# vlongle/pixie

Measured on NVIDIA H100. Metric: unet_voxels_per_s, higher is better.
Workload: dtype fp16e5 (U-Net, fp32 accumulate) + f32 (MPM)

## Files before the change

### pixie_b200/csrc/capi.cu

```cuda
#include "../../include/pixie_b200.h"
#include "mpm.cuh"
#include "unet.cuh"
#include "unet_kernels.cuh"
#include "field_transfer.cuh"
#include "cluster.cuh"
#include "particle_fill.cuh"
#include "nearest.cuh"
#include "gs_render.cuh"
#include "gs_ply.cuh"
#include "gs_load.cuh"
#include "material_metrics.cuh"
#include "part_segmentation.cuh"
#include "workspace.cuh"

#include <algorithm>
#include <cstring>
#include <string>

namespace {
thread_local std::string g_err;
}

namespace pixie {
int fail(const std::string& message) { g_err = message; return 1; }
int fail(const std::string& what, cudaError_t e) {
    cudaGetLastError();
    return fail(what + ": " + cudaGetErrorString(e));
}
}

using pixie::fail;

namespace {
int check(const char* op, cudaError_t e) { return e == cudaSuccess ? 0 : fail(op, e); }
}

extern "C" {

const char* pixie_last_error(void) { return g_err.c_str(); }
int pixie_abi_version(void) { return 2; }

int pixie_device_ok(void) {
    int dev = 0;
    if (cudaGetDevice(&dev) != cudaSuccess) { cudaGetLastError(); return 0; }
    int major = 0;
    if (cudaDeviceGetAttribute(&major, cudaDevAttrComputeCapabilityMajor, dev) != cudaSuccess) { cudaGetLastError(); return 0; }
    return major == 9 ? 1 : 0;
}

static int require_device() {
    if (!pixie_device_ok()) return fail("pixie_b200 requires an sm_90 (H100) CUDA device; there is no CPU fallback");
    return 0;
}

int pixie_unet_create(const pixie_unet_config* cfg, pixie_unet_t* out) {
    if (!cfg || !out) return fail("null argument");
    if (require_device()) return 1;
    *out = pixie::unet_create(*cfg);
    return *out ? 0 : 1;
}
int pixie_unet_set_tensor(pixie_unet_t h, const char* name, const float* host_data, const int64_t* shape, int ndim) {
    if (!h || !name || !host_data) return fail("null argument");
    return pixie::unet_set_tensor(h, name, host_data, shape, ndim);
}
int pixie_unet_finalize(pixie_unet_t h) {
    if (!h) return fail("null handle");
    return pixie::unet_finalize(h);
}
int pixie_unet_forward(pixie_unet_t h, const void* feat, int batch, float* out, void* stream) {
    if (!h || !feat || !out) return fail("null argument");
    return pixie::unet_forward(h, feat, batch, out, (cudaStream_t)stream);
}
int pixie_unet_forward_ncdhw(pixie_unet_t h, const float* feat, int batch, float* out, void* stream) {
    if (!h || !feat || !out) return fail("null argument");
    return pixie::unet_forward_ncdhw(h, feat, batch, out, (cudaStream_t)stream);
}
int pixie_unet_forward_host(pixie_unet_t h, const void* feat, int batch, float* out, void* stream) {
    if (!h || !feat || !out) return fail("null argument");
    return pixie::unet_forward_host(h, feat, batch, out, (cudaStream_t)stream);
}
int pixie_unet_profile(pixie_unet_t h, const void* feat, int batch, float* out, void* stream, float* ms, int* kinds, double* flops, int cap) {
    if (!h || !feat || !out || !ms || !kinds || !flops) { fail("null argument"); return -1; }
    return pixie::unet_profile(h, feat, batch, out, (cudaStream_t)stream, ms, kinds, flops, cap);
}
int pixie_field_extract(const float* pred, int n_classes, const float* mask, int D, const double ranges[6], const double bmin[3], const double bmax[3],
                        float* pos, float* density, float* E, float* nu, int* material, float* conf, int* count_host, void* stream) {
    if (!pred || !mask || !ranges || !bmin || !bmax || !pos || !density || !E || !nu || !material || !conf || !count_host) return fail("null argument");
    if (D < 2 || D > 1290 || n_classes < 1)
        return fail("field_extract: need 2 <= D <= 1290 (D^3 voxels are indexed in int32) and at least one class channel");
    if (require_device()) return 1;
    return check("field_extract", pixie::field_extract(pred, n_classes, mask, D, ranges, bmin, bmax, pos, density, E, nu, material, conf,
                                                       count_host, (cudaStream_t)stream));
}
int pixie_knn_assign(const float* query, int nq, const float* pos, const float* density, const float* E, const float* nu, const int* material,
                     const int* part, const float* conf, int m, int k, double threshold, int weighted, const float defaults[4], int def_material,
                     int def_part, float* o_density, float* o_E, float* o_nu, int* o_material, int* o_part, float* o_conf, int* n_too_far_host,
                     void* stream) {
    if (!query || !pos || !density || !E || !nu || !material || !part || !conf || !defaults || !o_density || !o_E || !o_nu || !o_material ||
        !o_part || !o_conf || !n_too_far_host) return fail("null argument");
    if (k < 1 || k > 16) return fail("knn_assign: k must be in [1, 16]");
    if (m < 1) return fail("knn_assign: empty material point cloud");
    if (k > m) return fail("knn_assign: k exceeds the number of material points");
    if (require_device()) return 1;
    return check("knn_assign", pixie::knn_assign(query, nq, pos, density, E, nu, material, part, conf, m, k, threshold, weighted, defaults,
                                                 def_material, def_part, o_density, o_E, o_nu, o_material, o_part, o_conf, n_too_far_host,
                                                 (cudaStream_t)stream));
}
int pixie_dbscan(const float* pos, int n, const int* ids, int select_id, double eps, int min_samples, int* index, int* labels,
                 int* n_selected_host, int* n_clusters_host, void* stream) {
    if (!n_selected_host || !n_clusters_host || (n > 0 && (!pos || !index || !labels))) return fail("null argument");
    if (n < 0) return fail("dbscan: negative point count");
    if (!(eps > 0.0) || min_samples < 1) return fail("dbscan: need eps > 0 and min_samples >= 1");
    if (require_device()) return 1;
    return check("dbscan", pixie::dbscan(pos, n, ids, select_id, eps, min_samples, index, labels, n_selected_host, n_clusters_host,
                                         (cudaStream_t)stream));
}
int pixie_cluster_stats(const float* pos, const int* index, const int* labels, int n_selected, int n_clusters, int* sizes,
                        float* bbox_min, float* bbox_max, void* stream) {
    if (n_selected < 0 || n_clusters < 0) return fail("cluster_stats: negative count");
    if ((n_selected > 0 && (!pos || !index || !labels)) || (n_clusters > 0 && (!sizes || !bbox_min || !bbox_max))) return fail("null argument");
    if (require_device()) return 1;
    return check("cluster_stats", pixie::cluster_stats(pos, index, labels, n_selected, n_clusters, sizes, bbox_min, bbox_max, (cudaStream_t)stream));
}
int pixie_particle_volume(const float* pos, int n, int grid_n, float grid_dx, float* vol, void* stream) {
    if (n < 0) return fail("particle_volume: negative point count");
    if (n > 0 && (!pos || !vol)) return fail("null argument");
    if (grid_n < 1 || !(grid_dx > 0.f)) return fail("particle_volume: bad grid");
    if (require_device()) return 1;
    return check("particle_volume", pixie::particle_volume(pos, n, grid_n, grid_dx, vol, (cudaStream_t)stream));
}
int pixie_frame_transform(const float* pos, const float* cov, int n, float z_shift, float scale, const float mean[3], const float* rotations,
                          int n_rot, float* pos_out, float* cov_out, void* stream) {
    if (n < 0) return fail("frame_transform: negative point count");
    if (!mean || (n > 0 && (!pos || !pos_out || (cov && !cov_out))) || (n_rot > 0 && !rotations)) return fail("null argument");
    if (n_rot < 0 || n_rot > 8) return fail("frame_transform: at most 8 rotations");
    if (require_device()) return 1;
    return check("frame_transform", pixie::frame_transform(pos, cov, n, z_shift, scale, mean, rotations, n_rot, pos_out, cov_out, (cudaStream_t)stream));
}
int pixie_gaussian_ply_records(const float* pos, const float* cov, const float* shs, int K, const float* opacity, int n, float* records,
                               void* stream) {
    if (n < 0) return fail("gaussian_ply_records: negative point count");
    if (K != 1 && K != 4 && K != 9 && K != 16) return fail("gaussian_ply_records: K must be 1, 4, 9 or 16 SH coefficients");
    if (n > 0 && (!pos || !cov || !shs || !opacity || !records)) return fail("null argument");
    if (require_device()) return 1;
    return check("gaussian_ply_records", pixie::gaussian_ply_records(pos, cov, shs, K, opacity, n, records, (cudaStream_t)stream));
}
int pixie_gaussian_checkpoint_decode(const void* table, long long n, int row_bytes, const int* cols, int K, int has_threshold, float threshold,
                                     float* pos, float* shs, float* opacity, float* cov, long long* m_host, void* stream) {
    if (!cols || !m_host || (n > 0 && (!table || !pos || !shs || !opacity || !cov))) return fail("null argument");
    if (n < 0) return fail("gaussian_checkpoint_decode: negative row count");
    if (K != 1 && K != 4 && K != 9 && K != 16) return fail("gaussian_checkpoint_decode: K must be 1, 4, 9 or 16 SH coefficients");
    if (row_bytes < 4 || row_bytes % 4 != 0 || row_bytes / 4 > pixie::kGsLoadMaxRowWords)
        return fail("gaussian_checkpoint_decode: the row stride must be a multiple of 4 bytes, at most " +
                       std::to_string(4 * pixie::kGsLoadMaxRowWords));
    const int row_words = row_bytes / 4, n_cols = 11 + 3 * K;
    pixie::GsColumns c{};
    int* dst[59];
    int k = 0;
    for (int i = 0; i < 3; ++i) dst[k++] = &c.xyz[i];
    for (int i = 0; i < 3; ++i) dst[k++] = &c.dc[i];
    for (int i = 0; i < 3 * (K - 1); ++i) dst[k++] = &c.rest[i];
    dst[k++] = &c.opacity;
    for (int i = 0; i < 3; ++i) dst[k++] = &c.scale[i];
    for (int i = 0; i < 4; ++i) dst[k++] = &c.rot[i];
    for (int i = 0; i < n_cols; ++i) {
        if (cols[i] < 0 || cols[i] % 4 != 0 || cols[i] / 4 >= row_words)
            return fail("gaussian_checkpoint_decode: column " + std::to_string(i) + " is not a 4-byte aligned offset inside the row");
        *dst[i] = cols[i] / 4;
    }
    if (require_device()) return 1;
    return check("gaussian_checkpoint_decode", pixie::gaussian_checkpoint_decode(table, n, row_words, c, K, has_threshold, threshold, pos, shs, opacity,
                                                                                 cov, m_host, (cudaStream_t)stream));
}
int pixie_material_metrics(const float* mat, int c_mat, const float* mask, const float* seg, int n_classes, const float* cont, int n,
                           int64_t voxels, const double* ranges, int background_id, float* gt, long long* counts, double* sums, void* stream) {
    if (!ranges || (n > 0 && (!mat || !seg || !cont || !gt || !counts || !sums))) return fail("null argument");
    if (n < 0 || voxels < 1) return fail("material_metrics: need n >= 0 samples of at least one voxel");
    if (c_mat < 4) return fail("material_metrics: the material grid needs at least 4 channels (density, E, nu, ..., material id)");
    if (n_classes < 1) return fail("material_metrics: need at least one class");
    pixie::MaterialNorm nm;
    for (int c = 0; c < 3; ++c) {
        const double lo = ranges[2 * c], hi = ranges[2 * c + 1];
        nm.lo[c] = (float)lo;
        nm.hi[c] = (float)hi;
        nm.span[c] = (float)(hi - lo);
    }
    if (require_device()) return 1;
    return check("material_metrics", pixie::material_metrics(mat, c_mat, mask, seg, n_classes, cont, n, voxels, nm, background_id, gt, counts, sums,
                                                             (cudaStream_t)stream));
}
static bool fill_grid_ok(int grid_n) { return grid_n >= 1 && grid_n <= 1290; }
int pixie_fill_density(const float* pos, const float* opacity, const float* cov, int n, int grid_n, float grid_dx, int* count, float* density,
                       void* stream) {
    if (!count || !density || (n > 0 && (!pos || !opacity || !cov))) return fail("null argument");
    if (n < 0 || !fill_grid_ok(grid_n) || !(grid_dx > 0.f)) return fail("fill_density: need n >= 0, 1 <= grid_n <= 1290 and grid_dx > 0");
    if (require_device()) return 1;
    return check("fill_density", pixie::fill_density(pos, opacity, cov, n, grid_n, grid_dx, count, density, (cudaStream_t)stream));
}
int pixie_fill_grids(int* count, const float* density, int grid_n, float grid_dx, const float origin[3], float density_thres, float search_thres,
                     int max_particles_per_cell, int exclude_dir, int ray_cast_dir, unsigned long long seed, float* out, int max_samples,
                     int* n_dense_host, int* n_total_host, void* stream) {
    if (!count || !density || !origin || !n_dense_host || !n_total_host || (max_samples > 0 && !out)) return fail("null argument");
    if (!fill_grid_ok(grid_n) || !(grid_dx > 0.f)) return fail("fill_grids: need 1 <= grid_n <= 1290 and grid_dx > 0");
    if (max_particles_per_cell < 1 || (long long)grid_n * grid_n * grid_n * max_particles_per_cell > 2147483647LL)
        return fail("fill_grids: need 1 <= max_particles_per_cell and grid_n^3 * max_particles_per_cell < 2^31");
    if (exclude_dir < 0 || exclude_dir > 5 || ray_cast_dir < 0 || ray_cast_dir > 5) return fail("fill_grids: directions must be in 0..5");
    if (max_samples < 0) return fail("fill_grids: negative max_samples");
    if (require_device()) return 1;
    if (check("fill_grids", pixie::fill_grids(count, density, grid_n, grid_dx, origin, density_thres, search_thres, max_particles_per_cell,
                                              exclude_dir, ray_cast_dir, seed, out, max_samples, n_dense_host, n_total_host, (cudaStream_t)stream)))
        return 1;
    if (*n_total_host > max_samples)
        return fail("fill_grids: filling adds " + std::to_string(*n_total_host) + " particles (" + std::to_string(*n_dense_host) +
                       " in dense cells) but max_samples is " + std::to_string(max_samples));
    return 0;
}
int pixie_nearest_gaussian(const float* pos, int n, const float* query, int m, int* index, void* stream) {
    if (n < 0 || m < 0) return fail("nearest_gaussian: negative count");
    if ((n > 0 && m > 0 && !pos) || (m > 0 && (!query || !index))) return fail("null argument");
    if (require_device()) return 1;
    return check("nearest_gaussian", pixie::nearest_gaussian(pos, n, query, m, index, (cudaStream_t)stream));
}
int pixie_nearest_vertex(const double* vert, int n, const float* query, int m, int* index, void* stream) {
    if (n < 0 || m < 0) return fail("nearest_vertex: negative count");
    if ((n > 0 && m > 0 && !vert) || (m > 0 && (!query || !index))) return fail("null argument");
    if (require_device()) return 1;
    return check("nearest_vertex", pixie::nearest_vertex(vert, n, query, m, index, (cudaStream_t)stream));
}
int pixie_knn_label_vote(const float* pos, int n, const int64_t* labels, int k, int64_t* out, void* stream) {
    if (n < 0) return fail("knn_label_vote: negative count");
    if (n > 0 && (k < 1 || k > n)) return fail("knn_label_vote: k must be in [1, n]");
    if (n > 0 && (!pos || !labels || !out)) return fail("null argument");
    if (require_device()) return 1;
    return check("knn_label_vote", pixie::knn_label_vote(pos, n, (const long long*)labels, k, (long long*)out, (cudaStream_t)stream));
}
int pixie_part_similarity(const void* feat, const uint8_t* mask, int64_t n_voxels, int C, int n_occupied, const float* query, int P,
                          float inv_temperature, float* sims, int64_t* labels, float* scores, float* probs, void* stream) {
    if (n_voxels < 0 || n_occupied < 0) return fail("part_similarity: negative count");
    if (n_voxels > INT32_MAX) return fail("part_similarity: more than 2^31 - 1 voxels");
    if (C < 1) return fail("part_similarity: C must be >= 1");
    if (P < 1 || P > pixie::kMaxParts) return fail("part_similarity: P must be in [1, " + std::to_string(pixie::kMaxParts) + "]");
    if (n_occupied > n_voxels) return fail("part_similarity: more occupied voxels than voxels");
    if (n_occupied > 0 && (!feat || !query || !sims || !labels || !scores)) return fail("null argument");
    if (require_device()) return 1;
    return check("part_similarity", pixie::part_similarity((const __half*)feat, mask, n_voxels, C, n_occupied, query, P, inv_temperature,
                                                           sims, labels, scores, probs, (cudaStream_t)stream));
}
int pixie_gs_renderer_create(pixie_gs_renderer_t* out) {
    if (!out) return fail("null argument");
    if (require_device()) return 1;
    *out = pixie::gs_renderer_create();
    return *out ? 0 : 1;
}
int pixie_gs_render(pixie_gs_renderer_t h, const float* means, const float* cov, const float* opacity, const float* shs, int sh_coeffs,
                    int sh_degree, const float* colors, int n, const float view[16], const float proj[16], const float campos[3],
                    float tan_fovx, float tan_fovy, int width, int height, const float bg[3], float* image, int* radii, int* n_rendered,
                    float* phase_ms, void* stream) {
    if (!h) return fail("null handle");
    if (!view || !proj || !campos || !bg || !image || (n > 0 && (!means || !cov || !opacity || !radii || (!shs && !colors))))
        return fail("null argument");
    if (n < 0) return fail("gs_render: negative Gaussian count");
    if (width < 1 || height < 1 || (long long)width * height > 2147483647LL) return fail("gs_render: bad image size");
    if (!(tan_fovx > 0.f) || !(tan_fovy > 0.f)) return fail("gs_render: tan(fov) must be positive");
    if (shs && (sh_degree < 0 || sh_degree > 3 || (sh_degree + 1) * (sh_degree + 1) > sh_coeffs))
        return fail("gs_render: need 0 <= sh_degree <= 3 and (sh_degree + 1)^2 <= sh_coeffs");
    pixie::GsRenderArgs a{};
    a.means = means; a.cov = cov; a.opacity = opacity; a.shs = shs; a.colors = shs ? nullptr : colors;
    a.n = n; a.sh_coeffs = sh_coeffs; a.sh_degree = sh_degree;
    std::memcpy(a.view, view, sizeof(a.view));
    std::memcpy(a.proj, proj, sizeof(a.proj));
    std::memcpy(a.campos, campos, sizeof(a.campos));
    std::memcpy(a.bg, bg, sizeof(a.bg));
    a.tan_fovx = tan_fovx; a.tan_fovy = tan_fovy; a.width = width; a.height = height; a.image = image; a.radii = radii;
    return pixie::gs_render(h, a, n_rendered, phase_ms, (cudaStream_t)stream);
}
void pixie_gs_renderer_destroy(pixie_gs_renderer_t h) { pixie::gs_renderer_destroy(h); }
int pixie_pack_predictions(const float* seg_logits_dev, const float* cont_dev, float* out_dev, int batch, int64_t voxels, int n_classes, void* stream) {
    if (!seg_logits_dev || !cont_dev || !out_dev) return fail("null argument");
    if (require_device()) return 1;
    return check("pack_predictions",
                 (cudaError_t)pixie::launch_pack_predictions(seg_logits_dev, cont_dev, out_dev, batch, voxels, n_classes, (cudaStream_t)stream));
}
int pixie_unet_launch_count(pixie_unet_t h) { return h ? pixie::unet_launch_count(h) : 0; }
double pixie_unet_flops(pixie_unet_t h) { return h ? pixie::unet_flops(h) : 0.0; }
int pixie_unet_check(pixie_unet_t h) {
    if (!h) return fail("null handle");
    return pixie::unet_check(h);
}
int64_t pixie_unet_debug_fetch(pixie_unet_t h, const char* name, float* host_out, int64_t capacity) {
    if (!h || !name) { fail("null argument"); return -1; }
    return pixie::unet_debug_fetch(h, name, host_out, capacity);
}
int64_t pixie_unet_debug_names(pixie_unet_t h, char* buf, int64_t capacity) {
    if (!h || (!buf && capacity > 0)) { fail("null argument"); return -1; }
    const std::string s = pixie::unet_debug_names(h);
    if (capacity > 0) {
        const size_t n = std::min(s.size(), (size_t)capacity - 1);
        memcpy(buf, s.data(), n);
        buf[n] = '\0';
    }
    return (int64_t)s.size();
}
void pixie_unet_destroy(pixie_unet_t h) { pixie::unet_destroy(h); }

int pixie_mpm_create(int n_particles, int n_grid, float grid_lim, pixie_mpm_t* out) {
    if (!out) return fail("null argument");
    if (require_device()) return 1;
    *out = pixie::mpm_create(n_particles, n_grid, grid_lim);
    return *out ? 0 : 1;
}
int pixie_mpm_bind(pixie_mpm_t h, int field, void* dev_ptr) { return h ? pixie::mpm_bind(h, field, dev_ptr) : fail("null handle"); }
int pixie_mpm_set_params(pixie_mpm_t h, const pixie_mpm_params* p) { return !p ? fail("null params") : h ? pixie::mpm_set_params(h, *p) : fail("null handle"); }
int pixie_mpm_add_bc(pixie_mpm_t h, const pixie_mpm_bc* bc) { return !bc ? fail("null bc") : h ? pixie::mpm_add_bc(h, *bc) : fail("null handle"); }
int pixie_mpm_clear_bcs(pixie_mpm_t h) { return h ? pixie::mpm_clear_bcs(h) : fail("null handle"); }
int pixie_mpm_set_time(pixie_mpm_t h, double t) { return h ? pixie::mpm_set_time(h, t) : fail("null handle"); }
int pixie_mpm_get_time(pixie_mpm_t h, double* t) { return h ? pixie::mpm_get_time(h, t) : fail("null handle"); }
int pixie_mpm_step(pixie_mpm_t h, int n, double dt, void* stream) { return h ? pixie::mpm_step(h, n, dt, (cudaStream_t)stream) : fail("null handle"); }
int pixie_mpm_compute_mu_lam(pixie_mpm_t h, void* s) { return h ? pixie::mpm_compute_mu_lam(h, (cudaStream_t)s) : fail("null handle"); }
int pixie_mpm_compute_bulk(pixie_mpm_t h, void* s) { return h ? pixie::mpm_compute_bulk(h, (cudaStream_t)s) : fail("null handle"); }
int pixie_mpm_compute_mass(pixie_mpm_t h, void* s) { return h ? pixie::mpm_compute_mass(h, (cudaStream_t)s) : fail("null handle"); }
int pixie_mpm_compute_cov_from_F(pixie_mpm_t h, void* s) { return h ? pixie::mpm_compute_cov_from_F(h, (cudaStream_t)s) : fail("null handle"); }
int pixie_mpm_compute_R_from_F(pixie_mpm_t h, void* s) { return h ? pixie::mpm_compute_R_from_F(h, (cudaStream_t)s) : fail("null handle"); }
int pixie_mpm_apply_additional_params(pixie_mpm_t h, const float* boxes, int n_boxes, void* s) {
    return h ? pixie::mpm_apply_additional_params(h, boxes, n_boxes, (cudaStream_t)s) : fail("null handle");
}
int pixie_mpm_select_box(pixie_mpm_t h, const float point[3], const float size[3], int* mask, void* s) {
    return h ? pixie::mpm_select_box(h, point, size, mask, (cudaStream_t)s) : fail("null handle");
}
int pixie_mpm_select_cylinder(pixie_mpm_t h, const float point[3], const float normal[3], float hh, float radius, int* mask, void* s) {
    return h ? pixie::mpm_select_cylinder(h, point, normal, hh, radius, mask, (cudaStream_t)s) : fail("null handle");
}
int pixie_mpm_sync(pixie_mpm_t h, void* s) { return h ? pixie::mpm_sync(h, (cudaStream_t)s) : fail("null handle"); }
int pixie_mpm_set_active_count(pixie_mpm_t h, int n_active) { return h ? pixie::mpm_set_active_count(h, n_active) : fail("null handle"); }
int pixie_mpm_grid_ptrs(pixie_mpm_t h, float** mv4, float** v4) { return h ? pixie::mpm_grid_ptrs(h, mv4, v4) : fail("null handle"); }
int pixie_mpm_exchange_buffer(pixie_mpm_t h, void** base, size_t* bytes) { return h ? pixie::mpm_exchange_buffer(h, base, bytes) : fail("null handle"); }
int pixie_mpm_slab_attach(pixie_mpm_t h, int x0, int x1, int slack, const void* left, const void* right) {
    return h ? pixie::mpm_slab_attach(h, x0, x1, slack, left, right) : fail("null handle");
}
int pixie_mpm_slab_phase(pixie_mpm_t h, int phase, double dt, void* s) { return h ? pixie::mpm_slab_phase(h, phase, dt, (cudaStream_t)s) : fail("null handle"); }
int pixie_mpm_slab_error(pixie_mpm_t h, int* flag) { return h ? pixie::mpm_slab_error(h, flag) : fail("null handle"); }
int pixie_mpm_slab_excursion(pixie_mpm_t h, int* d_out, void* s) { return h ? pixie::mpm_slab_excursion(h, d_out, (cudaStream_t)s) : fail("null handle"); }
int pixie_ipc_export(const void* dev_ptr, unsigned char handle[64]) {
    static_assert(sizeof(cudaIpcMemHandle_t) == 64, "cudaIpcMemHandle_t size");
    cudaIpcMemHandle_t hd;
    if (check("cudaIpcGetMemHandle", cudaIpcGetMemHandle(&hd, const_cast<void*>(dev_ptr)))) return 1;
    memcpy(handle, &hd, 64);
    return 0;
}
int pixie_ipc_open(const unsigned char handle[64], void** dev_ptr) {
    cudaIpcMemHandle_t hd;
    memcpy(&hd, handle, 64);
    return check("cudaIpcOpenMemHandle", cudaIpcOpenMemHandle(dev_ptr, hd, cudaIpcMemLazyEnablePeerAccess));
}
int pixie_ipc_close(void* dev_ptr) { return check("cudaIpcCloseMemHandle", cudaIpcCloseMemHandle(dev_ptr)); }
long long pixie_mpm_launch_count(pixie_mpm_t h) { return h ? pixie::mpm_launch_count(h) : 0; }
void pixie_mpm_destroy(pixie_mpm_t h) { pixie::mpm_destroy(h); }

}
```

### pixie_b200/csrc/conv3d_igemm.cu

```cuda
#include "conv3d_igemm.cuh"
#include "ptx.cuh"

#include <algorithm>
#include <cmath>
#include <cstdio>
#include <cstring>

#include <cuda_fp8.h>

namespace pixie {

using namespace ptx;

namespace {

constexpr int kMaxWStages = 4;
constexpr int kMaxSStages = 8;
constexpr int kConsumerWarps = 8;
constexpr int kProducerWarp = 8;

struct SmemCtrl {
    uint64_t wfull[kMaxWStages];
    uint64_t wempty[kMaxWStages];
    uint64_t sfull[kMaxSStages];
    uint64_t sempty[kMaxSStages];
    int abort_flag;
};

constexpr int kCtlBarrierBytes = 512;
constexpr int kCmChunk = 16;
constexpr int kCmStageLd = 68;
constexpr int kCmStageFloats = kCmChunk * kCmStageLd;
constexpr int kStatsMaxC = 256;

struct TileCoord {
    int nb, d0, h0, w0, n0, ph_begin, ph_end, split, tde;
};

__device__ __forceinline__ TileCoord decode_tile(const ConvKernelParams& p, int wi) {
    TileCoord t;
    unsigned rest = (unsigned)wi;
    if (p.split_k == 1) {
        t.split = 0; t.ph_begin = 0; t.ph_end = p.n_phases;
    } else {
        const unsigned sk = (unsigned)p.split_k;
        t.split = (int)(rest % sk);
        rest /= sk;
        t.ph_begin = (int)(((unsigned)t.split * (unsigned)p.n_phases) / sk);
        t.ph_end = (int)((((unsigned)t.split + 1u) * (unsigned)p.n_phases) / sk);
    }
    const unsigned nt = rest % (unsigned)p.n_tiles;
    unsigned m = rest / (unsigned)p.n_tiles;
    const unsigned tw = m % (unsigned)p.tiles_w;
    m /= (unsigned)p.tiles_w;
    const unsigned th = m % (unsigned)p.tiles_h;
    m /= (unsigned)p.tiles_h;
    const unsigned td = m % (unsigned)p.tiles_d;
    t.nb = (int)(m / (unsigned)p.tiles_d);
    t.d0 = (int)td * p.TD;
    t.h0 = (int)th * p.TH;
    t.w0 = (int)tw * p.TW;
    t.n0 = (int)nt * p.block_n;
    t.tde = min(p.TD, p.D - t.d0);
    return t;
}

template <int N, bool F8>
__device__ __forceinline__ void mma_block(float* acc, uint32_t a, uint32_t b) {
    wgmma_fence();
#pragma unroll
    for (int k4 = 0; k4 < 4; ++k4) {
        const uint64_t da = make_sw128_desc(a + 32u * k4), db = make_sw128_desc(b + 32u * k4);
        if (F8) {
            if (N == 16) wgmma_e5m2_n16(acc, da, db);
            if (N == 32) wgmma_e5m2_n32(acc, da, db);
            if (N == 64) wgmma_e5m2_n64(acc, da, db);
            if (N == 128) wgmma_e5m2_n128(acc, da, db);
            if (N == 256) wgmma_e5m2_n256(acc, da, db);
        } else {
            if (N == 16) wgmma_f16_n16(acc, da, db);
            if (N == 32) wgmma_f16_n32(acc, da, db);
            if (N == 64) wgmma_f16_n64(acc, da, db);
            if (N == 128) wgmma_f16_n128(acc, da, db);
            if (N == 256) wgmma_f16_n256(acc, da, db);
        }
    }
    wgmma_commit();
}

__device__ __forceinline__ void wgmma_wait_n(int n) {
    switch (n) {
        case 0: wgmma_wait<0>(); break;
        case 1: wgmma_wait<1>(); break;
        case 2: wgmma_wait<2>(); break;
        case 3: wgmma_wait<3>(); break;
        case 4: wgmma_wait<4>(); break;
        case 5: wgmma_wait<5>(); break;
        case 6: wgmma_wait<6>(); break;
        case 7: wgmma_wait<7>(); break;
        case 8: wgmma_wait<8>(); break;
        case 9: wgmma_wait<9>(); break;
        default: wgmma_wait<0>(); break;
    }
}

struct RingPos {
    int stage = 0, parity = 0;
    __device__ __forceinline__ void advance(int n_stages) {
        if (++stage == n_stages) { stage = 0; parity ^= 1; }
    }
};

struct PendingStages {
    int s = -1, w = -1;
    __device__ __forceinline__ void release(SmemCtrl* ctl, int lane) {
        if (lane == 0) {
            if (s >= 0) mbar_arrive(&ctl->sempty[s]);
            if (w >= 0) mbar_arrive(&ctl->wempty[w]);
        }
        s = -1; w = -1;
    }
};

struct ConvStats {
    float* rows;
    int nb = -1;
    double tot_s = 0.0, tot_q = 0.0;

    __device__ __forceinline__ void flush(const ConvKernelParams& p, int lane) {
        if (p.stats_scalar) {
#pragma unroll
            for (int off = 16; off >= 1; off >>= 1) {
                tot_s += __shfl_xor_sync(0xffffffffu, tot_s, off);
                tot_q += __shfl_xor_sync(0xffffffffu, tot_q, off);
            }
            if (lane == 0) {
                atomicAdd(p.stats + (size_t)nb * p.Cout * 2, tot_s);
                atomicAdd(p.stats + (size_t)nb * p.Cout * 2 + 1, tot_q);
            }
            tot_s = 0.0; tot_q = 0.0;
            return;
        }
        asm volatile("bar.sync 1, 256;" ::: "memory");
        for (int ch = threadIdx.x; ch < p.Cout; ch += 256) {
            atomicAdd(p.stats + ((size_t)nb * p.Cout + ch) * 2, (double)rows[ch]);
            atomicAdd(p.stats + ((size_t)nb * p.Cout + ch) * 2 + 1, (double)rows[p.stats_ld + ch]);
            rows[ch] = 0.f;
            rows[p.stats_ld + ch] = 0.f;
        }
        asm volatile("bar.sync 1, 256;" ::: "memory");
    }
    __device__ __forceinline__ void enter(const ConvKernelParams& p, int item_nb, int lane) {
        if (nb != item_nb) {
            if (nb >= 0) flush(p, lane);
            nb = item_nb;
        }
    }
};

struct ConvSmem {
    uint8_t* w;
    uint8_t* s;
    SmemCtrl* ctl;
    float* stage;
    float* stats;
};

__device__ __forceinline__ ConvSmem conv_prologue(const ConvKernelParams& p, int stage_floats, int n_threads) {
    extern __shared__ __align__(1024) uint8_t smem_raw[];
    uint8_t* smem = reinterpret_cast<uint8_t*>(
        (reinterpret_cast<uintptr_t>(smem_raw) + 1023) & ~static_cast<uintptr_t>(1023));
    ConvSmem m;
    m.w = smem;
    m.s = smem + (size_t)p.w_stages * p.w_stage_bytes;
    m.ctl = reinterpret_cast<SmemCtrl*>(m.s + (size_t)p.s_stages * p.s_stage_bytes);
    m.stage = reinterpret_cast<float*>(reinterpret_cast<uint8_t*>(m.ctl) + kCtlBarrierBytes);
    m.stats = m.stage + stage_floats;
    const bool smem_misaligned = (p.smem_slack == 0) && (smem != smem_raw);

    if (threadIdx.x == 0) {
        for (int i = 0; i < kMaxWStages; ++i) { mbar_init(&m.ctl->wfull[i], 1); mbar_init(&m.ctl->wempty[i], kConsumerWarps); }
        for (int i = 0; i < kMaxSStages; ++i) { mbar_init(&m.ctl->sfull[i], 1); mbar_init(&m.ctl->sempty[i], kConsumerWarps); }
        m.ctl->abort_flag = smem_misaligned ? 1 : 0;
        fence_barrier_init();
    }
    if ((threadIdx.x >> 5) == kProducerWarp && (threadIdx.x & 31) == 0) {
        for (int i = 0; i < kConvMaxSrc; ++i) prefetch_tmap(&p.tmA[i]);
        prefetch_tmap(&p.tmB);
    }
    if (p.stats != nullptr && !p.stats_scalar)
        for (int i = threadIdx.x; i < 2 * p.stats_ld; i += n_threads) m.stats[i] = 0.f;
    __syncthreads();
    return m;
}

__device__ __forceinline__ void conv_report_abort(const ConvKernelParams& p, const SmemCtrl* ctl) {
    __syncthreads();
    if (threadIdx.x == 0 && ctl->abort_flag && p.err_flag) atomicExch(p.err_flag, 1 + (int)blockIdx.x);
}

template <int BN, int TD>
__device__ __forceinline__ int issue_slab(float (&acc)[TD][BN / 2], uint32_t a_addr, uint32_t w_addr, int pl, int d_min, int d_max,
                                          int n_kd, int n_kh, int TW, bool f8) {
    int groups = 0;
#pragma unroll
    for (int d = 0; d < TD; ++d) {
        if (d < d_min || d > d_max) continue;
        const int kd = pl - d;
        for (int kh = 0; kh < n_kh; ++kh) {
            const uint32_t a = a_addr + (uint32_t)(kh * TW * 128);
            const uint32_t b = w_addr + (uint32_t)(conv_wtile(0, n_kd, kh, kd) * BN * 128);
            if (f8) mma_block<BN, true>(acc[d], a, b);
            else mma_block<BN, false>(acc[d], a, b);
            ++groups;
        }
    }
    return groups;
}

constexpr int kWholePhase = 0;

template <int kUnitKd>
__device__ __forceinline__ void produce_tiles(const ConvKernelParams& p, SmemCtrl* ctl, uint8_t* w_smem, uint8_t* s_smem,
                                              volatile int* abort_flag, int total_items) {
    RingPos wring, sring;
    bool ok = true;
    for (int wi = blockIdx.x; wi < total_items && ok; wi += gridDim.x) {
        const TileCoord t = decode_tile(p, wi);
        for (int ph = t.ph_begin; ph < t.ph_end && ok; ++ph) {
            const ConvPhase P = p.phases[ph];
            const int n_kd = P.n_kd, n_kh = P.n_kh, nplanes = t.tde + n_kd - 1;
            const int unit_kd = kUnitKd ? kUnitKd : n_kd, n_units = kUnitKd ? n_kd / kUnitKd : 1;
            const uint32_t slab_bytes = (uint32_t)p.slab_rows[P.src] * 128u, unit_bytes = (uint32_t)(n_kh * unit_kd * p.block_n * 128);
            const CUtensorMap* tm = &p.tmA[P.src];
            const int cw = t.w0 * p.stride + P.dw, ch = t.h0 * p.stride + P.dh0, cd = t.d0 * p.stride + P.dd0;
#pragma unroll 1
            for (int pl = 0; pl < nplanes && ok; ++pl) {
                if (pl < n_units) {
                    ok = mbar_wait(&ctl->wempty[wring.stage], wring.parity ^ 1, abort_flag);
                    if (!ok) break;
                    if (elect_one()) {
                        mbar_expect_tx(&ctl->wfull[wring.stage], unit_bytes);
                        uint8_t* wdst = w_smem + (size_t)wring.stage * p.w_stage_bytes;
                        const int kd_lo = pl * unit_kd, kd_hi = kd_lo + unit_kd - 1;
#pragma unroll 1
                        for (int kh = 0; kh < n_kh; ++kh)
                            for (int kd = kd_hi; kd >= kd_lo; --kd)
                                tma_load_2d(wdst + (size_t)conv_wtile(0, unit_kd, kh, kd - kd_lo) * p.block_n * 128, &p.tmB,
                                            &ctl->wfull[wring.stage], conv_wtile(P.wtile_base, n_kd, kh, kd) * 64, t.n0);
                    }
                    wring.advance(p.w_stages);
                }
                ok = mbar_wait(&ctl->sempty[sring.stage], sring.parity ^ 1, abort_flag);
                if (!ok) break;
                if (elect_one()) {
                    mbar_expect_tx(&ctl->sfull[sring.stage], slab_bytes);
                    tma_load_5d(s_smem + (size_t)sring.stage * p.s_stage_bytes, tm, &ctl->sfull[sring.stage], (int)P.c0, cw, ch,
                                cd + pl * p.stride, t.nb);
                }
                sring.advance(p.s_stages);
            }
        }
    }
}

}

template <int BN, int TD>
__global__ void __launch_bounds__(kConvThreads, 1)
conv3d_igemm_kernel(const __grid_constant__ ConvKernelParams p) {
    const ConvSmem sm = conv_prologue(p, 0, kConvThreads);
    SmemCtrl* ctl = sm.ctl;
    volatile int* abort_flag = &ctl->abort_flag;
    const int warp = threadIdx.x >> 5;
    const int lane = threadIdx.x & 31;
    const int total_items = conv_work_items(p.NB, p.tiles_d, p.tiles_h, p.tiles_w, p.n_tiles, p.split_k);
    const bool do_stats = p.stats != nullptr;
    const bool scalar_stats = do_stats && p.stats_scalar;

    if (warp == kProducerWarp) {
        produce_tiles<kWholePhase>(p, ctl, sm.w, sm.s, abort_flag, total_items);
    } else {
        const int g = warp >> 2, wq = warp & 3;
        float acc[TD][BN / 2];
        RingPos wring, sring;
        const uint32_t w_base0 = smem_u32(sm.w), s_base0 = smem_u32(sm.s) + (uint32_t)(g * 64 * 128);
        bool ok = true;
        const long long DHW = (long long)p.D * p.H * p.W;
        ConvStats stats{sm.stats};
        int th2[2], tw2[2];
#pragma unroll
        for (int r2 = 0; r2 < 2; ++r2) {
            const int r = g * 64 + wq * 16 + (lane >> 2) + 8 * r2;
            th2[r2] = r / p.TW; tw2[r2] = r % p.TW;
        }
        const int cq = (lane & 3) * 2;

        for (int wi = blockIdx.x; wi < total_items && ok; wi += gridDim.x) {
            const TileCoord t = decode_tile(p, wi);
#pragma unroll
            for (int d = 0; d < TD; ++d)
#pragma unroll
                for (int j = 0; j < BN / 2; ++j) acc[d][j] = 0.f;
            PendingStages pend;
            int prev_f8 = -1;
            for (int ph = t.ph_begin; ph < t.ph_end && ok; ++ph) {
                const ConvPhase P = p.phases[ph];
                const int n_kd = P.n_kd, n_kh = P.n_kh;
                const bool f8 = P.f8 != 0;
                if (prev_f8 >= 0 && prev_f8 != (int)f8) wgmma_wait<0>();
                prev_f8 = (int)f8;
                ok = mbar_wait(&ctl->wfull[wring.stage], wring.parity, abort_flag);
                if (!ok) break;
                const uint32_t w_addr = w_base0 + (uint32_t)(wring.stage * p.w_stage_bytes);
                const int nplanes = t.tde + n_kd - 1;
                for (int pl = 0; pl < nplanes && ok; ++pl) {
                    ok = mbar_wait(&ctl->sfull[sring.stage], sring.parity, abort_flag);
                    if (!ok) break;
                    const int d_min = max(0, pl - (n_kd - 1)), d_max = min(t.tde - 1, pl);
                    const int groups = issue_slab<BN, TD>(acc, s_base0 + (uint32_t)(sring.stage * p.s_stage_bytes), w_addr, pl, d_min,
                                                          d_max, n_kd, n_kh, p.TW, f8);
                    wgmma_wait_n(groups);
                    pend.release(ctl, lane);
                    pend.s = sring.stage;
                    sring.advance(p.s_stages);
                }
                pend.w = wring.stage;
                wring.advance(p.w_stages);
                if (p.w_stages == 1) { wgmma_wait<0>(); pend.release(ctl, lane); }
            }
            wgmma_wait<0>();
            pend.release(ctl, lane);
#pragma unroll
            for (int d = 0; d < TD; ++d)
#pragma unroll
                for (int j = 0; j < BN / 2; ++j) fence_operand(acc[d][j]);
            if (!ok) break;

            if (do_stats) stats.enter(p, t.nb, lane);
            const bool first_split = (t.split == 0);
            const bool use_bias = first_split && p.bias != nullptr;
            const bool use_res = first_split && p.residual != nullptr;
#pragma unroll
            for (int d = 0; d < TD; ++d) {
                if (d >= t.tde) break;
#pragma unroll
                for (int r2 = 0; r2 < 2; ++r2) {
                    const int hh = t.h0 + th2[r2], ww = t.w0 + tw2[r2];
                    const bool row_ok = (hh < p.H) && (ww < p.W);
                    const long long vox = ((long long)(t.d0 + d) * p.H + hh) * p.W + ww;
#pragma unroll
                    for (int j8 = 0; j8 < BN / 8; ++j8) {
                        const int ch = t.n0 + j8 * 8 + cq;
                        float& a0 = acc[d][j8 * 4 + r2 * 2];
                        float& a1 = acc[d][j8 * 4 + r2 * 2 + 1];
                        const bool ok0 = row_ok && ch < p.Cout, ok1 = row_ok && ch + 1 < p.Cout;
                        float v0 = a0, v1 = a1;
                        if (use_bias) {
                            if (ok0) v0 += __ldg(p.bias + ch);
                            if (ok1) v1 += __ldg(p.bias + ch + 1);
                        }
                        if (p.out_planar) {
                            const long long i0 = ((long long)t.nb * p.Cout + ch) * DHW + vox;
                            if (ok0) {
                                if (use_res) v0 += p.residual[i0];
                                if (p.atomic_out) atomicAdd(p.out + i0, v0); else p.out[i0] = v0;
                            }
                            if (ok1) {
                                if (use_res) v1 += p.residual[i0 + DHW];
                                if (p.atomic_out) atomicAdd(p.out + i0 + DHW, v1); else p.out[i0 + DHW] = v1;
                            }
                        } else if (ok0) {
                            const long long base = ((long long)t.nb * DHW + vox) * p.out_ld + p.out_c0 + ch;
                            if (ok1 && (base & 1) == 0) {
                                if (use_res) {
                                    const float2 rv = __ldg(reinterpret_cast<const float2*>(p.residual + base));
                                    v0 += rv.x; v1 += rv.y;
                                }
                                if (p.atomic_out) red_add_v2(p.out + base, v0, v1);
                                else *reinterpret_cast<float2*>(p.out + base) = make_float2(v0, v1);
                            } else {
                                if (use_res) { v0 += p.residual[base]; if (ok1) v1 += p.residual[base + 1]; }
                                if (p.atomic_out) { atomicAdd(p.out + base, v0); if (ok1) atomicAdd(p.out + base + 1, v1); }
                                else { p.out[base] = v0; if (ok1) p.out[base + 1] = v1; }
                            }
                        }
                        a0 = ok0 ? v0 : 0.f;
                        a1 = ok1 ? v1 : 0.f;
                    }
                }
            }
            if (do_stats) {
                if (scalar_stats) {
                    float s = 0.f, q2 = 0.f;
#pragma unroll
                    for (int d = 0; d < TD; ++d)
#pragma unroll
                        for (int j = 0; j < BN / 2; ++j) { s += acc[d][j]; q2 = fmaf(acc[d][j], acc[d][j], q2); }
                    stats.tot_s += (double)s; stats.tot_q += (double)q2;
                } else {
#pragma unroll
                    for (int j8 = 0; j8 < BN / 8; ++j8)
#pragma unroll
                        for (int e = 0; e < 2; ++e) {
                            float s = 0.f, q2 = 0.f;
#pragma unroll
                            for (int d = 0; d < TD; ++d)
#pragma unroll
                                for (int r2 = 0; r2 < 2; ++r2) {
                                    const float v = acc[d][j8 * 4 + r2 * 2 + e];
                                    s += v; q2 = fmaf(v, v, q2);
                                }
#pragma unroll
                            for (int off = 4; off <= 16; off <<= 1) {
                                s += __shfl_xor_sync(0xffffffffu, s, off);
                                q2 += __shfl_xor_sync(0xffffffffu, q2, off);
                            }
                            const int ch = t.n0 + j8 * 8 + cq + e;
                            if (lane < 4 && ch < p.Cout) {
                                atomicAdd(stats.rows + ch, s);
                                atomicAdd(stats.rows + p.stats_ld + ch, q2);
                            }
                        }
                }
            }
        }
        if (do_stats && stats.nb >= 0 && ok) stats.flush(p, lane);
    }

    conv_report_abort(p, ctl);
}

template <int NV>
__global__ void __launch_bounds__(kConvCmThreads, 1)
conv3d_igemm_cm_kernel(const __grid_constant__ ConvKernelParams p) {
    constexpr int TW = NV == 64 ? 8 : 16;
    const ConvSmem sm = conv_prologue(p, 2 * kCmStageFloats, kConvCmThreads);
    SmemCtrl* ctl = sm.ctl;
    volatile int* abort_flag = &ctl->abort_flag;
    const int warp = threadIdx.x >> 5;
    const int lane = threadIdx.x & 31;
    const int total_items = conv_work_items(p.NB, p.tiles_d, p.tiles_h, p.tiles_w, p.n_tiles, p.split_k);
    const bool do_stats = p.stats != nullptr;
    const bool scalar_stats = do_stats && p.stats_scalar;

    if (warp >= kProducerWarp) {
        setmaxnreg_dec<NV == 256 ? 40 : 56>();
        if (warp == kProducerWarp) produce_tiles<1>(p, ctl, sm.w, sm.s, abort_flag, total_items);
    } else {
        setmaxnreg_inc<NV == 256 ? 232 : 216>();
        const int g = warp >> 2, wq = warp & 3, wt = threadIdx.x & 127;
        float acc[NV / 2];
        RingPos wring, sring;
        const uint32_t w_base0 = smem_u32(sm.w), s_base0 = smem_u32(sm.s);
        bool ok = true;
        ConvStats stats{sm.stats};
        const int q4 = wt & 15, vr = wt >> 4;
        float* stage = sm.stage + g * kCmStageFloats;

        for (int wi = blockIdx.x; wi < total_items && ok; wi += gridDim.x) {
            const TileCoord t = decode_tile(p, wi);
#pragma unroll
            for (int j = 0; j < NV / 2; ++j) acc[j] = 0.f;
            const bool has_plane = g < t.tde;
            PendingStages pend;
            int prev_f8 = -1;
            for (int ph = t.ph_begin; ph < t.ph_end && ok; ++ph) {
                const ConvPhase P = p.phases[ph];
                const int n_kd = P.n_kd, n_kh = P.n_kh;
                const bool f8 = P.f8 != 0;
                if (prev_f8 >= 0 && prev_f8 != (int)f8) wgmma_wait<0>();
                prev_f8 = (int)f8;
                const int w0 = wring.stage;
                const int nplanes = t.tde + n_kd - 1;
                for (int pl = 0; pl < nplanes && ok; ++pl) {
                    if (pl < n_kd) {
                        ok = mbar_wait(&ctl->wfull[wring.stage], wring.parity, abort_flag);
                        if (!ok) break;
                        wring.advance(p.w_stages);
                    }
                    ok = mbar_wait(&ctl->sfull[sring.stage], sring.parity, abort_flag);
                    if (!ok) break;
                    const int kd = pl - g;
                    int groups = 0;
                    if (has_plane && kd >= 0 && kd < n_kd) {
                        int wsk = w0 + kd;
                        if (wsk >= p.w_stages) wsk -= p.w_stages;
                        const uint32_t w_addr = w_base0 + (uint32_t)(wsk * p.w_stage_bytes);
                        const uint32_t s_addr = s_base0 + (uint32_t)(sring.stage * p.s_stage_bytes);
                        for (int kh = 0; kh < n_kh; ++kh) {
                            const uint32_t a = w_addr + (uint32_t)(conv_wtile(0, 1, kh, 0) * 64 * 128);
                            const uint32_t b = s_addr + (uint32_t)(kh * TW * 128);
                            if (f8) mma_block<NV, true>(acc, a, b);
                            else mma_block<NV, false>(acc, a, b);
                            ++groups;
                        }
                    }
                    wgmma_wait_n(groups);
                    pend.release(ctl, lane);
                    pend.s = sring.stage;
                    const int kd_done = pl - t.tde + 1;
                    if (kd_done >= 0) {
                        pend.w = w0 + kd_done;
                        if (pend.w >= p.w_stages) pend.w -= p.w_stages;
                    }
                    sring.advance(p.s_stages);
                }
            }
            wgmma_wait<0>();
            pend.release(ctl, lane);
#pragma unroll
            for (int j = 0; j < NV / 2; ++j) fence_operand(acc[j]);
            if (!ok) break;

            if (do_stats) stats.enter(p, t.nb, lane);
            if (!has_plane) continue;
            const bool first_split = (t.split == 0);
            const int ch = t.n0 + 4 * q4;
            const bool ch_ok = ch < p.Cout;
            float4 bias4 = make_float4(0.f, 0.f, 0.f, 0.f);
            if (first_split && p.bias != nullptr && ch_ok)
                bias4 = make_float4(__ldg(p.bias + ch), __ldg(p.bias + ch + 1), __ldg(p.bias + ch + 2), __ldg(p.bias + ch + 3));
            const bool use_res = first_split && p.residual != nullptr;
            const long long plane_base = ((long long)t.nb * p.D + t.d0 + g) * p.H;
            float st_s[4] = {0.f, 0.f, 0.f, 0.f}, st_q[4] = {0.f, 0.f, 0.f, 0.f};
#pragma unroll
            for (int c = 0; c < NV / kCmChunk; ++c) {
#pragma unroll
                for (int jj = 0; jj < kCmChunk / 8; ++jj)
#pragma unroll
                    for (int r2 = 0; r2 < 2; ++r2)
#pragma unroll
                        for (int e = 0; e < 2; ++e) {
                            const int row = wq * 16 + (lane >> 2) + 8 * r2, v = jj * 8 + (lane & 3) * 2 + e;
                            stage[v * kCmStageLd + row] = acc[(c * (kCmChunk / 8) + jj) * 4 + r2 * 2 + e];
                        }
                asm volatile("bar.sync %0, 128;" ::"r"(2 + g) : "memory");
#pragma unroll
                for (int k = 0; k < kCmChunk / 8; ++k) {
                    const int v = vr + 8 * k, vt = c * kCmChunk + v;
                    const int hh = t.h0 + vt / TW, ww = t.w0 + vt % TW;
                    float4 x = *reinterpret_cast<const float4*>(stage + v * kCmStageLd + 4 * q4);
                    if (ch_ok && hh < p.H && ww < p.W) {
                        const long long base = ((plane_base + hh) * p.W + ww) * p.out_ld + p.out_c0 + ch;
                        x.x += bias4.x; x.y += bias4.y; x.z += bias4.z; x.w += bias4.w;
                        if (use_res) {
                            const float4 rv = __ldg(reinterpret_cast<const float4*>(p.residual + base));
                            x.x += rv.x; x.y += rv.y; x.z += rv.z; x.w += rv.w;
                        }
                        if (p.atomic_out) red_add_v4(p.out + base, x.x, x.y, x.z, x.w);
                        else *reinterpret_cast<float4*>(p.out + base) = x;
                        st_s[0] += x.x; st_s[1] += x.y; st_s[2] += x.z; st_s[3] += x.w;
                        st_q[0] = fmaf(x.x, x.x, st_q[0]); st_q[1] = fmaf(x.y, x.y, st_q[1]);
                        st_q[2] = fmaf(x.z, x.z, st_q[2]); st_q[3] = fmaf(x.w, x.w, st_q[3]);
                    }
                }
                asm volatile("bar.sync %0, 128;" ::"r"(2 + g) : "memory");
            }
            if (do_stats) {
                if (scalar_stats) {
                    stats.tot_s += (double)(st_s[0] + st_s[1] + st_s[2] + st_s[3]);
                    stats.tot_q += (double)(st_q[0] + st_q[1] + st_q[2] + st_q[3]);
                } else {
#pragma unroll
                    for (int i = 0; i < 4; ++i) {
                        st_s[i] += __shfl_xor_sync(0xffffffffu, st_s[i], 16);
                        st_q[i] += __shfl_xor_sync(0xffffffffu, st_q[i], 16);
                    }
                    if (lane < 16 && ch_ok) {
#pragma unroll
                        for (int i = 0; i < 4; ++i) {
                            atomicAdd(stats.rows + ch + i, st_s[i]);
                            atomicAdd(stats.rows + p.stats_ld + ch + i, st_q[i]);
                        }
                    }
                }
            }
        }
        if (do_stats && stats.nb >= 0 && ok) stats.flush(p, lane);
    }

    conv_report_abort(p, ctl);
}


int conv_k_total(const ConvDesc& d) {
    int k = 0;
    for (const auto& s : d.segs) k += s.ks * s.ks * s.ks * d.srcs[s.src].C;
    return k;
}

struct SrcSlot { int src; int n_kh; };

static std::vector<SrcSlot> conv_src_slots(const ConvDesc& d) {
    std::vector<SrcSlot> slots;
    for (const auto& s : d.segs) {
        const int n_kh = (s.ks == 3 && d.stride == 1) ? 3 : 1;
        bool found = false;
        for (const auto& sl : slots) found |= (sl.src == s.src && sl.n_kh == n_kh);
        if (!found) slots.push_back({s.src, n_kh});
    }
    return slots;
}

static int conv_slot_of(const std::vector<SrcSlot>& slots, int src, int n_kh) {
    for (size_t i = 0; i < slots.size(); ++i)
        if (slots[i].src == src && slots[i].n_kh == n_kh) return (int)i;
    return -1;
}

struct PhaseRec {
    ConvPhase P;
    int seg;
};

static std::vector<PhaseRec> conv_phase_records(const ConvDesc& d) {
    std::vector<PhaseRec> recs;
    const auto slots = conv_src_slots(d);
    int wtile = 0;
    for (int si = 0; si < (int)d.segs.size(); ++si) {
        const auto& s = d.segs[si];
        const int chunks = d.srcs[s.src].C / 64;
        const int n_k = (s.ks == 3 && d.stride == 1) ? 3 : 1, n_ph = s.ks / n_k, pad = s.ks / 2;
        for (int c = 0; c < chunks; ++c)
            for (int kw = 0; kw < s.ks; ++kw)
                for (int kh = 0; kh < n_ph; ++kh)
                    for (int kd = 0; kd < n_ph; ++kd) {
                        ConvPhase P{};
                        P.src = (int8_t)conv_slot_of(slots, s.src, n_k);
                        P.dw = (int8_t)(kw - pad);
                        P.dh0 = (int8_t)(kh - pad);
                        P.dd0 = (int8_t)(kd - pad);
                        P.n_kh = (int8_t)n_k;
                        P.n_kd = (int8_t)n_k;
                        P.c0 = (int16_t)(c * 64);
                        P.wtile_base = wtile;
                        P.f8 = s.f8;
                        wtile += n_k * n_k;
                        recs.push_back({P, si});
                    }
    }
    auto rank = [&](const PhaseRec& r) {
        const auto& s = d.segs[r.seg];
        return s.f8 ? 0 : (s.lo || s.wlo) ? 1 : 2;
    };
    std::stable_sort(recs.begin(), recs.end(), [&](const PhaseRec& a, const PhaseRec& b) { return rank(a) < rank(b); });
    return recs;
}

std::vector<ConvPhase> conv_build_phases(const ConvDesc& d) {
    std::vector<ConvPhase> ph;
    for (const auto& r : conv_phase_records(d)) ph.push_back(r.P);
    return ph;
}

void conv_pack_weights(const ConvDesc& d, const std::vector<const float*>& seg_weights,
                       const std::vector<int>& seg_cin_real, std::vector<__half>& packed) {
    const int K = conv_k_total(d);
    packed.assign((size_t)d.Cout_pad * K, __float2half(0.f));
    const float up = (float)(1 << kF8Shift), down = 1.0f / up;
    auto e5m2 = [](float v) { return (uint8_t)__nv_cvt_float_to_fp8(v, __NV_SATFINITE, __NV_E5M2); };
    for (const auto& r : conv_phase_records(d)) {
        const ConvPhase& P = r.P;
        const auto& s = d.segs[r.seg];
        const int cin = seg_cin_real[r.seg];
        const int ks = s.ks, kv = ks * ks * ks, pad = ks / 2;
        const float* w = seg_weights[r.seg];
        for (int kh = 0; kh < P.n_kh; ++kh)
            for (int kd = 0; kd < P.n_kd; ++kd) {
                const int tile = conv_wtile(P.wtile_base, P.n_kd, kh, kd);
                const int tap = ((P.dd0 + pad + kd) * ks + P.dh0 + pad + kh) * ks + P.dw + pad;
                for (int co = 0; co < d.Cout; ++co) {
                    uint8_t* row8 = reinterpret_cast<uint8_t*>(&packed[(size_t)co * K + (size_t)tile * 64]);
                    for (int cil = 0; cil < 64; ++cil) {
                        const int ci = P.c0 + cil;
                        if (ci >= cin) continue;
                        float v = w[((size_t)co * cin + ci) * kv + tap];
                        if (s.f8) {
                            row8[cil] = e5m2(v * down);
                            row8[64 + cil] = e5m2((v - __half2float(__float2half(v))) * up);
                            continue;
                        }
                        if (s.wlo) v = v - __half2float(__float2half(v));
                        packed[(size_t)co * K + (size_t)tile * 64 + cil] = __float2half(v);
                    }
                }
            }
    }
}

static ConvKernelFn conv_kernel_for(int bn, int td) {
    switch (bn * 8 + td) {
        case 16 * 8 + 1: return conv3d_igemm_kernel<16, 1>;
        case 16 * 8 + 2: return conv3d_igemm_kernel<16, 2>;
        case 16 * 8 + 4: return conv3d_igemm_kernel<16, 4>;
        case 32 * 8 + 1: return conv3d_igemm_kernel<32, 1>;
        case 32 * 8 + 2: return conv3d_igemm_kernel<32, 2>;
        default: return conv3d_igemm_kernel<32, 4>;
    }
}

static ConvKernelFn conv_cm_kernel_for(int nv) {
    switch (nv) {
        case 64: return conv3d_igemm_cm_kernel<64>;
        case 128: return conv3d_igemm_cm_kernel<128>;
        default: return conv3d_igemm_cm_kernel<256>;
    }
}

typedef CUresult (*PFN_encodeTiled)(CUtensorMap*, CUtensorMapDataType, cuuint32_t, void*,
                                    const cuuint64_t*, const cuuint64_t*, const cuuint32_t*,
                                    const cuuint32_t*, CUtensorMapInterleave, CUtensorMapSwizzle,
                                    CUtensorMapL2promotion, CUtensorMapFloatOOBfill);

static PFN_encodeTiled get_encode_fn() {
    static PFN_encodeTiled fn = nullptr;
    if (!fn) {
        void* p = nullptr;
        cudaDriverEntryPointQueryResult qres;
        if (cudaGetDriverEntryPoint("cuTensorMapEncodeTiled", &p, cudaEnableDefault, &qres) == cudaSuccess &&
            qres == cudaDriverEntryPointSuccess)
            fn = reinterpret_cast<PFN_encodeTiled>(p);
    }
    return fn;
}


static int encode_a_maps(const ConvDesc& d, ConvKernelParams& p, PFN_encodeTiled enc, char* err, int errlen) {
    const auto slots = conv_src_slots(d);
    for (size_t i = 0; i < slots.size(); ++i) {
        const ConvSrc& s = d.srcs[slots[i].src];
        cuuint64_t gdim[5] = {(cuuint64_t)s.C, (cuuint64_t)s.Win, (cuuint64_t)s.Hin, (cuuint64_t)s.Din, (cuuint64_t)d.NB};
        cuuint64_t gstr[4] = {(cuuint64_t)s.C * 2, (cuuint64_t)s.Win * s.C * 2,
                              (cuuint64_t)s.Hin * s.Win * s.C * 2, (cuuint64_t)s.Din * s.Hin * s.Win * s.C * 2};
        cuuint32_t box[5] = {64, (cuuint32_t)(p.TW * d.stride), (cuuint32_t)((p.TH + slots[i].n_kh - 1) * d.stride), 1, 1};
        cuuint32_t estr[5] = {1, (cuuint32_t)d.stride, (cuuint32_t)d.stride, 1, 1};
        CUresult r = enc(&p.tmA[i], CU_TENSOR_MAP_DATA_TYPE_FLOAT16, 5, (void*)s.ptr, gdim, gstr, box, estr,
                         CU_TENSOR_MAP_INTERLEAVE_NONE, CU_TENSOR_MAP_SWIZZLE_128B,
                         CU_TENSOR_MAP_L2_PROMOTION_L2_256B, CU_TENSOR_MAP_FLOAT_OOB_FILL_NONE);
        if (r != CUDA_SUCCESS) { snprintf(err, errlen, "cuTensorMapEncodeTiled(A%zu) failed: %d", i, (int)r); return 1; }
    }
    for (size_t i = slots.size(); i < (size_t)kConvMaxSrc; ++i) p.tmA[i] = p.tmA[0];
    return 0;
}

int conv_plan_retarget(const ConvDesc& d, ConvPlan& plan, char* err, int errlen) {
    PFN_encodeTiled enc = get_encode_fn();
    if (!enc) { snprintf(err, errlen, "cuTensorMapEncodeTiled unavailable"); return 1; }
    return encode_a_maps(d, plan.p, enc, err, errlen);
}

static const char* cm_geometry(const ConvDesc& d, int sms, int max_kh, ConvKernelParams& p) {
    int nv = d.nv;
    if (nv && nv != 64 && nv != 128 && nv != 256) return "bad nv";
    if (!nv) {
        double best = -1.0;
        for (int v : {256, 128, 64}) {
            if (v != 64 && d.W < 16) continue;
            const int tw = v == 64 ? 8 : 16, th = v / tw;
            const int tx = (d.W + tw - 1) / tw, ty = (d.H + th - 1) / th;
            const long long tiles = conv_work_items(d.NB, (d.D + 1) / 2, ty, tx, (d.Cout_pad + 63) / 64, 1);
            const long long rounds = (tiles + sms - 1) / sms;
            const double sc = (double)tiles / (double)(rounds * sms) * (double)d.W * d.H / (double)(tx * tw * ty * th) *
                              std::pow(0.93, v == 256 ? 0 : v == 128 ? 1 : 2);
            if (sc > best) { best = sc; nv = v; }
        }
    }
    p.TW = nv == 64 ? 8 : 16;
    p.TH = nv / p.TW;
    p.TD = 2;
    p.block_n = 64;
    p.w_stage_bytes = max_kh * p.block_n * 128;
    return nullptr;
}

static bool cm_stages(const ConvKernelParams& p, int max_kd, int avail, int& ws, int& ss) {
    ws = std::max(2, max_kd);
    if (ws * p.w_stage_bytes + 2 * p.s_stage_bytes > avail) return false;
    ss = std::min(std::min(kMaxSStages, 6), (avail - ws * p.w_stage_bytes) / p.s_stage_bytes);
    ws = std::min(kMaxWStages, (avail - ss * p.s_stage_bytes) / p.w_stage_bytes);
    return true;
}

static const char* vm_geometry(const ConvDesc& d, int sms, bool any3, int max_taps, ConvKernelParams& p) {
    p.TW = (d.W >= 16) ? 16 : 8;
    p.TH = 128 / p.TW;
    int bn = d.block_n;
    if (bn == 0) bn = d.Cout_pad > 16 ? 32 : 16;
    if (bn != 16 && bn != 32) return "bad block_n";

    int td = d.td ? d.td : std::min(4, 128 / bn);
    td = std::max(1, std::min(td, d.D));
    if (!any3 && !d.td) td = std::min(td, 2);
    if (td == 3) td = 2;
    if (td * bn > 128) return "TD*block_n exceeds the register accumulator budget (128)";
    if (!d.td && td > 1) {
        auto fill = [&](int t) {
            const long long tiles = conv_work_items(d.NB, (d.D + t - 1) / t, (d.H + p.TH - 1) / p.TH, (d.W + p.TW - 1) / p.TW,
                                                    (d.Cout_pad + bn - 1) / bn, 1);
            const long long rounds = (tiles + sms - 1) / sms;
            return (double)tiles / (double)(rounds * sms) * (t == td ? 1.0 : 0.93);
        };
        if (fill(td / 2) > fill(td)) td /= 2;
    }
    p.TD = td;
    p.block_n = bn;
    p.w_stage_bytes = max_taps * bn * 128;
    return nullptr;
}

static bool vm_stages(const ConvKernelParams& p, int avail, int& ws, int& ss) {
    ws = (2 * p.w_stage_bytes + 2 * p.s_stage_bytes <= avail) ? 2 : 1;
    if (ws * p.w_stage_bytes + 2 * p.s_stage_bytes > avail) return false;
    ss = std::min(std::min(kMaxSStages, 6), (avail - ws * p.w_stage_bytes) / p.s_stage_bytes);
    return true;
}

int conv_plan_create(const ConvDesc& d, int* d_err_flag, ConvPlan& plan, char* err, int errlen) {
    auto fail = [&](const char* m) { snprintf(err, errlen, "conv_plan_create: %s", m); return 1; };
    PFN_encodeTiled enc = get_encode_fn();
    if (!enc) return fail("cuTensorMapEncodeTiled unavailable (no CUDA driver?)");
    if (d.srcs.empty() || d.segs.empty()) return fail("no sources/segments");
    for (const auto& s : d.srcs)
        if (s.C % 64) return fail("source channels must be a multiple of 64");
    if (d.Cout_pad % 16 || d.Cout_pad < d.Cout) return fail("Cout_pad must be a multiple of 16 >= Cout");

    ConvKernelParams& p = plan.p;
    memset(&p, 0, sizeof(p));
    p.NB = d.NB; p.D = d.D; p.H = d.H; p.W = d.W; p.stride = d.stride;
    p.Cout = d.Cout;
    const int out_ld = d.out_ld ? d.out_ld : d.Cout;

    const auto slots = conv_src_slots(d);
    if ((int)slots.size() > kConvMaxSrc) return fail("too many (source, tap-class) slots");
    const std::vector<ConvPhase> phases = conv_build_phases(d);
    p.n_phases = (int)phases.size();
    int max_taps = 1, max_kh = 1, max_kd = 1;
    bool any3 = false;
    for (const auto& P : phases) {
        max_taps = std::max(max_taps, P.n_kh * P.n_kd);
        max_kh = std::max(max_kh, (int)P.n_kh);
        max_kd = std::max(max_kd, (int)P.n_kd);
        any3 |= (P.n_kh == 3);
    }

    int dev = 0, sms = 132;
    cudaGetDevice(&dev);
    cudaDeviceGetAttribute(&sms, cudaDevAttrMultiProcessorCount, dev);

    plan.channel_major = d.Cout >= 64 && d.Cout % 4 == 0 && !d.out_planar && out_ld % 4 == 0 && d.out_c0 % 4 == 0 &&
                         reinterpret_cast<uintptr_t>(d.out) % 16 == 0 && reinterpret_cast<uintptr_t>(d.residual) % 16 == 0;
    const char* bad = plan.channel_major ? cm_geometry(d, sms, max_kh, p) : vm_geometry(d, sms, any3, max_taps, p);
    if (bad) return fail(bad);
    p.n_tiles = (d.Cout_pad + p.block_n - 1) / p.block_n;
    p.tiles_w = (d.W + p.TW - 1) / p.TW;
    p.tiles_h = (d.H + p.TH - 1) / p.TH;
    p.tiles_d = (d.D + p.TD - 1) / p.TD;

    const int items = conv_work_items(d.NB, p.tiles_d, p.tiles_h, p.tiles_w, p.n_tiles, 1);
    int split = d.split_k;
    if (split <= 0) {
        split = 1;
        while (items * split < 120 && split * 2 <= p.n_phases && split < 64) split *= 2;
    }
    split = std::max(1, std::min(split, p.n_phases));
    if ((long long)p.n_phases * (split + 1) >= (1ll << 31)) return fail("too many phases for the split-K bookkeeping");
    p.split_k = split;
    p.atomic_out = split > 1;
    plan.needs_zero = split > 1;

    for (size_t i = 0; i < slots.size(); ++i) p.slab_rows[i] = p.TW * (p.TH + slots[i].n_kh - 1);
    int max_rows = 0;
    for (size_t i = 0; i < slots.size(); ++i) max_rows = std::max(max_rows, p.slab_rows[i]);
    p.s_stage_bytes = max_rows * 128;
    plan.fused_stats = d.stats != nullptr && split == 1 && d.Cout <= kStatsMaxC && !d.out_planar;
    p.stats_ld = (d.Cout + 31) / 32 * 32;
    const int stats_bytes = plan.fused_stats ? 2 * p.stats_ld * 4 : 0;
    const int ctl_core = kCtlBarrierBytes + (plan.channel_major ? 2 * kCmStageFloats * 4 : 0) + stats_bytes;
    auto plan_stages = [&](int slack, int& ws, int& ss) {
        const int avail = 227 * 1024 - ctl_core - slack;
        return plan.channel_major ? cm_stages(p, max_kd, avail, ws, ss) : vm_stages(p, avail, ws, ss);
    };
    int ws1 = 0, ss1 = 0, ws0 = 0, ss0 = 0;
    const bool ok1 = plan_stages(1024, ws1, ss1), ok0 = plan_stages(0, ws0, ss0);
    if (!ok0) return fail("tile does not fit in shared memory");
    if (ok1 && ws1 >= ws0 && ss1 >= ss0) { p.smem_slack = 1024; p.w_stages = ws1; p.s_stages = ss1; }
    else { p.smem_slack = 0; p.w_stages = ws0; p.s_stages = ss0; }
    const int ctl_bytes = ctl_core + p.smem_slack;
    plan.smem_bytes = p.w_stages * p.w_stage_bytes + p.s_stages * p.s_stage_bytes + ctl_bytes;

    if (encode_a_maps(d, p, enc, err, errlen)) return 1;
    {
        const int K = conv_k_total(d);
        cuuint64_t gdim[2] = {(cuuint64_t)K, (cuuint64_t)d.Cout_pad};
        cuuint64_t gstr[1] = {(cuuint64_t)K * 2};
        cuuint32_t box[2] = {64, (cuuint32_t)p.block_n};
        cuuint32_t estr[2] = {1, 1};
        CUresult r = enc(&p.tmB, CU_TENSOR_MAP_DATA_TYPE_FLOAT16, 2, (void*)d.weights, gdim, gstr, box, estr,
                         CU_TENSOR_MAP_INTERLEAVE_NONE, CU_TENSOR_MAP_SWIZZLE_128B,
                         CU_TENSOR_MAP_L2_PROMOTION_L2_256B, CU_TENSOR_MAP_FLOAT_OOB_FILL_NONE);
        if (r != CUDA_SUCCESS) { snprintf(err, errlen, "cuTensorMapEncodeTiled(B) failed: %d", (int)r); return 1; }
    }

    if (cudaMalloc(&plan.d_phases, phases.size() * sizeof(ConvPhase)) != cudaSuccess) return fail("cudaMalloc phases");
    cudaMemcpy(plan.d_phases, phases.data(), phases.size() * sizeof(ConvPhase), cudaMemcpyHostToDevice);
    p.phases = plan.d_phases;

    p.bias = d.bias; p.residual = d.residual; p.out = d.out;
    p.out_ld = out_ld; p.out_c0 = d.out_c0; p.out_planar = d.out_planar;
    p.err_flag = d_err_flag;
    p.stats = plan.fused_stats ? d.stats : nullptr;
    p.stats_scalar = d.stats_scalar ? 1 : 0;
    plan.out_item_bytes = d.out_planar ? (size_t)d.Cout * d.D * d.H * d.W * 4
                                       : (size_t)d.D * d.H * d.W * p.out_ld * 4;

    plan.grid = std::min(items * split, sms);

    plan.kernel = plan.channel_major ? conv_cm_kernel_for(p.TH * p.TW) : conv_kernel_for(p.block_n, p.TD);
    plan.threads = plan.channel_major ? kConvCmThreads : kConvThreads;
    if (cudaFuncSetAttribute(plan.kernel, cudaFuncAttributeMaxDynamicSharedMemorySize, 227 * 1024) != cudaSuccess)
        return fail("cudaFuncSetAttribute(max dynamic smem)");
    return 0;
}

void conv_plan_destroy(ConvPlan& plan) {
    if (plan.d_phases) cudaFree(plan.d_phases);
    plan.d_phases = nullptr;
}

int conv_plan_launch(const ConvPlan& plan, int nb, cudaStream_t stream) {
    if (nb < 1 || nb > plan.p.NB) return (int)cudaErrorInvalidValue;
    ConvKernelParams p = plan.p;
    p.NB = nb;
    const int grid = std::min(plan.grid, conv_work_items(nb, p.tiles_d, p.tiles_h, p.tiles_w, p.n_tiles, p.split_k));
    if (plan.needs_zero) cudaMemsetAsync(p.out, 0, plan.out_item_bytes * (size_t)nb, stream);
    plan.kernel<<<grid, plan.threads, plan.smem_bytes, stream>>>(p);
    return (int)cudaGetLastError();
}

}
```

### pixie_b200/csrc/conv3d_igemm.cuh

```cuda
#pragma once
#include <cuda.h>
#include <cuda_runtime.h>
#include <cuda_fp16.h>
#include <cstdint>
#include <vector>

namespace pixie {

constexpr int kConvMaxSrc = 8;
constexpr int kF8Shift = 6;
constexpr int kConvThreads = 288;
constexpr int kConvCmThreads = 384;

struct ConvPhase {
    int8_t src;
    int8_t dw;
    int8_t dh0;
    int8_t dd0;
    int8_t n_kh;
    int8_t n_kd;
    int16_t c0;
    int32_t wtile_base;
    int32_t f8;
};
static_assert(sizeof(ConvPhase) == 16, "ConvPhase layout");

__host__ __device__ __forceinline__ int conv_wtile(int wtile_base, int n_kd, int kh, int kd) {
    return wtile_base + kh * n_kd + (n_kd - 1 - kd);
}

__host__ __device__ __forceinline__ int conv_work_items(int nb, int tiles_d, int tiles_h, int tiles_w, int n_tiles, int split_k) {
    return nb * tiles_d * tiles_h * tiles_w * n_tiles * split_k;
}

struct ConvKernelParams {
    CUtensorMap tmA[kConvMaxSrc];
    CUtensorMap tmB;
    const ConvPhase* phases;
    int n_phases;
    int split_k;
    int NB, D, H, W;
    int stride;
    int TW, TH, TD;
    int tiles_w, tiles_h, tiles_d;
    int Cout;
    int block_n;
    int n_tiles;
    int w_stage_bytes, w_stages;
    int s_stage_bytes, s_stages;
    int slab_rows[kConvMaxSrc];
    const float* bias;
    const float* residual;
    float* out;
    int out_ld;
    int out_c0;
    int out_planar;
    int atomic_out;
    double* stats;
    int stats_ld;
    int smem_slack;
    int stats_scalar;
    int* err_flag;
};

typedef void (*ConvKernelFn)(ConvKernelParams);

struct ConvSrc {
    const __half* ptr;
    int C;
    int Din, Hin, Win;
};

struct ConvDesc {
    int NB = 1;
    int D = 0, H = 0, W = 0;
    int stride = 1;
    int Cout = 0;
    struct Seg { int src; int ks; int wlo = 0; int f8 = 0; int lo = 0; };
    std::vector<ConvSrc> srcs;
    std::vector<Seg> segs;
    const __half* weights = nullptr;
    int Cout_pad = 0;
    const float* bias = nullptr;
    const float* residual = nullptr;
    float* out = nullptr;
    int out_ld = 0, out_c0 = 0, out_planar = 0;
    double* stats = nullptr;
    bool stats_scalar = false;
    int split_k = 1;
    int block_n = 0;
    int td = 0;
    int nv = 0;
};

int conv_k_total(const ConvDesc& d);

std::vector<ConvPhase> conv_build_phases(const ConvDesc& d);

void conv_pack_weights(const ConvDesc& d, const std::vector<const float*>& seg_weights,
                       const std::vector<int>& seg_cin_real, std::vector<__half>& packed);

struct ConvPlan {
    ConvKernelParams p{};
    ConvPhase* d_phases = nullptr;
    ConvKernelFn kernel = nullptr;
    bool channel_major = false;
    int threads = 0;
    int grid = 0;
    int smem_bytes = 0;
    bool needs_zero = false;
    bool fused_stats = false;
    size_t out_item_bytes = 0;
};

int conv_plan_create(const ConvDesc& d, int* d_err_flag, ConvPlan& plan, char* err, int errlen);
void conv_plan_destroy(ConvPlan& plan);
int conv_plan_launch(const ConvPlan& plan, int nb, cudaStream_t stream);
int conv_plan_retarget(const ConvDesc& d, ConvPlan& plan, char* err, int errlen);
}
```

### pixie_b200/csrc/ptx.cuh

```cuda
#pragma once
#include <cstdint>
#include <cuda_runtime.h>

namespace pixie {
namespace ptx {

__device__ __forceinline__ uint32_t smem_u32(const void* p) {
    return static_cast<uint32_t>(__cvta_generic_to_shared(p));
}

__device__ __forceinline__ bool elect_one() {
    uint32_t pred = 0;
    asm volatile(
        "{\n\t"
        ".reg .pred P;\n\t"
        "elect.sync _|P, 0xffffffff;\n\t"
        "selp.u32 %0, 1, 0, P;\n\t"
        "}\n"
        : "=r"(pred));
    return pred != 0;
}

__device__ __forceinline__ void mbar_init(uint64_t* bar, uint32_t count) {
    asm volatile("mbarrier.init.shared::cta.b64 [%0], %1;" ::"r"(smem_u32(bar)), "r"(count));
}
__device__ __forceinline__ void fence_barrier_init() {
    asm volatile("fence.mbarrier_init.release.cluster;" ::: "memory");
}
__device__ __forceinline__ void fence_proxy_async() {
    asm volatile("fence.proxy.async.shared::cta;" ::: "memory");
}
__device__ __forceinline__ void mbar_expect_tx(uint64_t* bar, uint32_t bytes) {
    asm volatile("mbarrier.arrive.expect_tx.shared::cta.b64 _, [%0], %1;" ::"r"(smem_u32(bar)),
                 "r"(bytes)
                 : "memory");
}
__device__ __forceinline__ void mbar_arrive(uint64_t* bar) {
    asm volatile("mbarrier.arrive.shared::cta.b64 _, [%0];" ::"r"(smem_u32(bar)) : "memory");
}
__device__ __forceinline__ bool mbar_try_wait(uint64_t* bar, uint32_t parity) {
    uint32_t ok;
    asm volatile(
        "{\n\t"
        ".reg .pred P;\n\t"
        "mbarrier.try_wait.parity.shared::cta.b64 P, [%1], %2;\n\t"
        "selp.u32 %0, 1, 0, P;\n\t"
        "}\n"
        : "=r"(ok)
        : "r"(smem_u32(bar)), "r"(parity)
        : "memory");
    return ok != 0;
}
__device__ __forceinline__ bool mbar_wait(uint64_t* bar, uint32_t parity, volatile int* abort_flag) {
    for (uint32_t it = 0; it < (1u << 22); ++it) {
        if (mbar_try_wait(bar, parity)) return true;
        if ((it & 1023u) == 1023u && *abort_flag) return false;
    }
    *abort_flag = 1;
    return false;
}

__device__ __forceinline__ void prefetch_tmap(const void* tmap) {
    asm volatile("prefetch.tensormap [%0];" ::"l"(reinterpret_cast<uint64_t>(tmap)) : "memory");
}
__device__ __forceinline__ void tma_load_2d(void* dst, const void* tmap, uint64_t* bar, int c0,
                                            int c1) {
    asm volatile(
        "cp.async.bulk.tensor.2d.shared::cluster.global.mbarrier::complete_tx::bytes"
        " [%0], [%1, {%3, %4}], [%2];"
        :
        : "r"(smem_u32(dst)), "l"(reinterpret_cast<uint64_t>(tmap)), "r"(smem_u32(bar)), "r"(c0),
          "r"(c1)
        : "memory");
}
__device__ __forceinline__ void tma_load_5d(void* dst, const void* tmap, uint64_t* bar, int c0,
                                            int c1, int c2, int c3, int c4) {
    asm volatile(
        "cp.async.bulk.tensor.5d.shared::cluster.global.mbarrier::complete_tx::bytes"
        " [%0], [%1, {%3, %4, %5, %6, %7}], [%2];"
        :
        : "r"(smem_u32(dst)), "l"(reinterpret_cast<uint64_t>(tmap)), "r"(smem_u32(bar)), "r"(c0),
          "r"(c1), "r"(c2), "r"(c3), "r"(c4)
        : "memory");
}

__device__ __forceinline__ void wgmma_fence() { asm volatile("wgmma.fence.sync.aligned;" ::: "memory"); }
__device__ __forceinline__ void wgmma_commit() { asm volatile("wgmma.commit_group.sync.aligned;" ::: "memory"); }
template <int N>
__device__ __forceinline__ void wgmma_wait() { asm volatile("wgmma.wait_group.sync.aligned %0;" ::"n"(N) : "memory"); }
__device__ __forceinline__ void fence_operand(float& r) { asm volatile("" : "+f"(r)::"memory"); }

__device__ __forceinline__ uint64_t make_sw128_desc(uint32_t smem_addr) {
    uint64_t d = 0;
    d |= static_cast<uint64_t>((smem_addr & 0x3FFFFu) >> 4);
    d |= static_cast<uint64_t>(1) << 16;
    d |= static_cast<uint64_t>(1024 >> 4) << 32;
    d |= static_cast<uint64_t>(1) << 62;
    return d;
}

__device__ __forceinline__ void wgmma_f16_n16(float* d, uint64_t da, uint64_t db) {
    asm volatile(
        "{\n\t.reg .pred p;\n\tsetp.ne.b32 p, %10, 0;\n\t"
        "wgmma.mma_async.sync.aligned.m64n16k16.f32.f16.f16 "
        "{%0, %1, %2, %3, %4, %5, %6, %7}, %8, %9, p, 1, 1, 0, 0;\n\t}\n"
        : "+f"(d[0]), "+f"(d[1]), "+f"(d[2]), "+f"(d[3]), "+f"(d[4]), "+f"(d[5]), "+f"(d[6]), "+f"(d[7])
        : "l"(da), "l"(db), "r"(1));
}
__device__ __forceinline__ void wgmma_f16_n32(float* d, uint64_t da, uint64_t db) {
    asm volatile(
        "{\n\t.reg .pred p;\n\tsetp.ne.b32 p, %18, 0;\n\t"
        "wgmma.mma_async.sync.aligned.m64n32k16.f32.f16.f16 "
        "{%0, %1, %2, %3, %4, %5, %6, %7, %8, %9, %10, %11, %12, %13, %14, %15}, %16, %17, p, 1, 1, 0, 0;\n\t}\n"
        : "+f"(d[0]), "+f"(d[1]), "+f"(d[2]), "+f"(d[3]), "+f"(d[4]), "+f"(d[5]), "+f"(d[6]), "+f"(d[7]), "+f"(d[8]), "+f"(d[9]), "+f"(d[10]), "+f"(d[11]), "+f"(d[12]), "+f"(d[13]), "+f"(d[14]), "+f"(d[15])
        : "l"(da), "l"(db), "r"(1));
}
__device__ __forceinline__ void wgmma_f16_n64(float* d, uint64_t da, uint64_t db) {
    asm volatile(
        "{\n\t.reg .pred p;\n\tsetp.ne.b32 p, %34, 0;\n\t"
        "wgmma.mma_async.sync.aligned.m64n64k16.f32.f16.f16 "
        "{%0, %1, %2, %3, %4, %5, %6, %7, %8, %9, %10, %11, %12, %13, %14, %15, %16, %17, %18, %19, %20, %21, %22, %23, %24, %25, %26, %27, %28, %29, %30, %31}, %32, %33, p, 1, 1, 0, 0;\n\t}\n"
        : "+f"(d[0]), "+f"(d[1]), "+f"(d[2]), "+f"(d[3]), "+f"(d[4]), "+f"(d[5]), "+f"(d[6]), "+f"(d[7]), "+f"(d[8]), "+f"(d[9]), "+f"(d[10]), "+f"(d[11]), "+f"(d[12]), "+f"(d[13]), "+f"(d[14]), "+f"(d[15]), "+f"(d[16]), "+f"(d[17]), "+f"(d[18]), "+f"(d[19]), "+f"(d[20]), "+f"(d[21]), "+f"(d[22]), "+f"(d[23]), "+f"(d[24]), "+f"(d[25]), "+f"(d[26]), "+f"(d[27]), "+f"(d[28]), "+f"(d[29]), "+f"(d[30]), "+f"(d[31])
        : "l"(da), "l"(db), "r"(1));
}
__device__ __forceinline__ void wgmma_e5m2_n16(float* d, uint64_t da, uint64_t db) {
    asm volatile(
        "{\n\t.reg .pred p;\n\tsetp.ne.b32 p, %10, 0;\n\t"
        "wgmma.mma_async.sync.aligned.m64n16k32.f32.e5m2.e5m2 "
        "{%0, %1, %2, %3, %4, %5, %6, %7}, %8, %9, p, 1, 1;\n\t}\n"
        : "+f"(d[0]), "+f"(d[1]), "+f"(d[2]), "+f"(d[3]), "+f"(d[4]), "+f"(d[5]), "+f"(d[6]), "+f"(d[7])
        : "l"(da), "l"(db), "r"(1));
}
__device__ __forceinline__ void wgmma_e5m2_n32(float* d, uint64_t da, uint64_t db) {
    asm volatile(
        "{\n\t.reg .pred p;\n\tsetp.ne.b32 p, %18, 0;\n\t"
        "wgmma.mma_async.sync.aligned.m64n32k32.f32.e5m2.e5m2 "
        "{%0, %1, %2, %3, %4, %5, %6, %7, %8, %9, %10, %11, %12, %13, %14, %15}, %16, %17, p, 1, 1;\n\t}\n"
        : "+f"(d[0]), "+f"(d[1]), "+f"(d[2]), "+f"(d[3]), "+f"(d[4]), "+f"(d[5]), "+f"(d[6]), "+f"(d[7]), "+f"(d[8]), "+f"(d[9]), "+f"(d[10]), "+f"(d[11]), "+f"(d[12]), "+f"(d[13]), "+f"(d[14]), "+f"(d[15])
        : "l"(da), "l"(db), "r"(1));
}
__device__ __forceinline__ void wgmma_e5m2_n64(float* d, uint64_t da, uint64_t db) {
    asm volatile(
        "{\n\t.reg .pred p;\n\tsetp.ne.b32 p, %34, 0;\n\t"
        "wgmma.mma_async.sync.aligned.m64n64k32.f32.e5m2.e5m2 "
        "{%0, %1, %2, %3, %4, %5, %6, %7, %8, %9, %10, %11, %12, %13, %14, %15, %16, %17, %18, %19, %20, %21, %22, %23, %24, %25, %26, %27, %28, %29, %30, %31}, %32, %33, p, 1, 1;\n\t}\n"
        : "+f"(d[0]), "+f"(d[1]), "+f"(d[2]), "+f"(d[3]), "+f"(d[4]), "+f"(d[5]), "+f"(d[6]), "+f"(d[7]), "+f"(d[8]), "+f"(d[9]), "+f"(d[10]), "+f"(d[11]), "+f"(d[12]), "+f"(d[13]), "+f"(d[14]), "+f"(d[15]), "+f"(d[16]), "+f"(d[17]), "+f"(d[18]), "+f"(d[19]), "+f"(d[20]), "+f"(d[21]), "+f"(d[22]), "+f"(d[23]), "+f"(d[24]), "+f"(d[25]), "+f"(d[26]), "+f"(d[27]), "+f"(d[28]), "+f"(d[29]), "+f"(d[30]), "+f"(d[31])
        : "l"(da), "l"(db), "r"(1));
}

__device__ __forceinline__ void wgmma_f16_n128(float* d, uint64_t da, uint64_t db) {
    asm volatile(
        "{\n\t.reg .pred p;\n\tsetp.ne.b32 p, %66, 0;\n\t"
        "wgmma.mma_async.sync.aligned.m64n128k16.f32.f16.f16 "
        "{%0, %1, %2, %3, %4, %5, %6, %7, %8, %9, %10, %11, %12, %13, %14, %15, %16, %17, %18, %19, %20, %21, %22, %23, %24, %25, %26, %27, %28, %29, %30, %31, %32, %33, %34, %35, %36, %37, %38, %39, %40, %41, %42, %43, %44, %45, %46, %47, %48, %49, %50, %51, %52, %53, %54, %55, %56, %57, %58, %59, %60, %61, %62, %63}, %64, %65, p, 1, 1, 0, 0;\n\t}\n"
        : "+f"(d[0]), "+f"(d[1]), "+f"(d[2]), "+f"(d[3]), "+f"(d[4]), "+f"(d[5]), "+f"(d[6]), "+f"(d[7]), "+f"(d[8]), "+f"(d[9]), "+f"(d[10]), "+f"(d[11]), "+f"(d[12]), "+f"(d[13]), "+f"(d[14]), "+f"(d[15]), "+f"(d[16]), "+f"(d[17]), "+f"(d[18]), "+f"(d[19]), "+f"(d[20]), "+f"(d[21]), "+f"(d[22]), "+f"(d[23]), "+f"(d[24]), "+f"(d[25]), "+f"(d[26]), "+f"(d[27]), "+f"(d[28]), "+f"(d[29]), "+f"(d[30]), "+f"(d[31]), "+f"(d[32]), "+f"(d[33]), "+f"(d[34]), "+f"(d[35]), "+f"(d[36]), "+f"(d[37]), "+f"(d[38]), "+f"(d[39]), "+f"(d[40]), "+f"(d[41]), "+f"(d[42]), "+f"(d[43]), "+f"(d[44]), "+f"(d[45]), "+f"(d[46]), "+f"(d[47]), "+f"(d[48]), "+f"(d[49]), "+f"(d[50]), "+f"(d[51]), "+f"(d[52]), "+f"(d[53]), "+f"(d[54]), "+f"(d[55]), "+f"(d[56]), "+f"(d[57]), "+f"(d[58]), "+f"(d[59]), "+f"(d[60]), "+f"(d[61]), "+f"(d[62]), "+f"(d[63])
        : "l"(da), "l"(db), "r"(1));
}
__device__ __forceinline__ void wgmma_f16_n256(float* d, uint64_t da, uint64_t db) {
    asm volatile(
        "{\n\t.reg .pred p;\n\tsetp.ne.b32 p, %130, 0;\n\t"
        "wgmma.mma_async.sync.aligned.m64n256k16.f32.f16.f16 "
        "{%0, %1, %2, %3, %4, %5, %6, %7, %8, %9, %10, %11, %12, %13, %14, %15, %16, %17, %18, %19, %20, %21, %22, %23, %24, %25, %26, %27, %28, %29, %30, %31, %32, %33, %34, %35, %36, %37, %38, %39, %40, %41, %42, %43, %44, %45, %46, %47, %48, %49, %50, %51, %52, %53, %54, %55, %56, %57, %58, %59, %60, %61, %62, %63, %64, %65, %66, %67, %68, %69, %70, %71, %72, %73, %74, %75, %76, %77, %78, %79, %80, %81, %82, %83, %84, %85, %86, %87, %88, %89, %90, %91, %92, %93, %94, %95, %96, %97, %98, %99, %100, %101, %102, %103, %104, %105, %106, %107, %108, %109, %110, %111, %112, %113, %114, %115, %116, %117, %118, %119, %120, %121, %122, %123, %124, %125, %126, %127}, %128, %129, p, 1, 1, 0, 0;\n\t}\n"
        : "+f"(d[0]), "+f"(d[1]), "+f"(d[2]), "+f"(d[3]), "+f"(d[4]), "+f"(d[5]), "+f"(d[6]), "+f"(d[7]), "+f"(d[8]), "+f"(d[9]), "+f"(d[10]), "+f"(d[11]), "+f"(d[12]), "+f"(d[13]), "+f"(d[14]), "+f"(d[15]), "+f"(d[16]), "+f"(d[17]), "+f"(d[18]), "+f"(d[19]), "+f"(d[20]), "+f"(d[21]), "+f"(d[22]), "+f"(d[23]), "+f"(d[24]), "+f"(d[25]), "+f"(d[26]), "+f"(d[27]), "+f"(d[28]), "+f"(d[29]), "+f"(d[30]), "+f"(d[31]), "+f"(d[32]), "+f"(d[33]), "+f"(d[34]), "+f"(d[35]), "+f"(d[36]), "+f"(d[37]), "+f"(d[38]), "+f"(d[39]), "+f"(d[40]), "+f"(d[41]), "+f"(d[42]), "+f"(d[43]), "+f"(d[44]), "+f"(d[45]), "+f"(d[46]), "+f"(d[47]), "+f"(d[48]), "+f"(d[49]), "+f"(d[50]), "+f"(d[51]), "+f"(d[52]), "+f"(d[53]), "+f"(d[54]), "+f"(d[55]), "+f"(d[56]), "+f"(d[57]), "+f"(d[58]), "+f"(d[59]), "+f"(d[60]), "+f"(d[61]), "+f"(d[62]), "+f"(d[63]), "+f"(d[64]), "+f"(d[65]), "+f"(d[66]), "+f"(d[67]), "+f"(d[68]), "+f"(d[69]), "+f"(d[70]), "+f"(d[71]), "+f"(d[72]), "+f"(d[73]), "+f"(d[74]), "+f"(d[75]), "+f"(d[76]), "+f"(d[77]), "+f"(d[78]), "+f"(d[79]), "+f"(d[80]), "+f"(d[81]), "+f"(d[82]), "+f"(d[83]), "+f"(d[84]), "+f"(d[85]), "+f"(d[86]), "+f"(d[87]), "+f"(d[88]), "+f"(d[89]), "+f"(d[90]), "+f"(d[91]), "+f"(d[92]), "+f"(d[93]), "+f"(d[94]), "+f"(d[95]), "+f"(d[96]), "+f"(d[97]), "+f"(d[98]), "+f"(d[99]), "+f"(d[100]), "+f"(d[101]), "+f"(d[102]), "+f"(d[103]), "+f"(d[104]), "+f"(d[105]), "+f"(d[106]), "+f"(d[107]), "+f"(d[108]), "+f"(d[109]), "+f"(d[110]), "+f"(d[111]), "+f"(d[112]), "+f"(d[113]), "+f"(d[114]), "+f"(d[115]), "+f"(d[116]), "+f"(d[117]), "+f"(d[118]), "+f"(d[119]), "+f"(d[120]), "+f"(d[121]), "+f"(d[122]), "+f"(d[123]), "+f"(d[124]), "+f"(d[125]), "+f"(d[126]), "+f"(d[127])
        : "l"(da), "l"(db), "r"(1));
}
__device__ __forceinline__ void wgmma_e5m2_n128(float* d, uint64_t da, uint64_t db) {
    asm volatile(
        "{\n\t.reg .pred p;\n\tsetp.ne.b32 p, %66, 0;\n\t"
        "wgmma.mma_async.sync.aligned.m64n128k32.f32.e5m2.e5m2 "
        "{%0, %1, %2, %3, %4, %5, %6, %7, %8, %9, %10, %11, %12, %13, %14, %15, %16, %17, %18, %19, %20, %21, %22, %23, %24, %25, %26, %27, %28, %29, %30, %31, %32, %33, %34, %35, %36, %37, %38, %39, %40, %41, %42, %43, %44, %45, %46, %47, %48, %49, %50, %51, %52, %53, %54, %55, %56, %57, %58, %59, %60, %61, %62, %63}, %64, %65, p, 1, 1;\n\t}\n"
        : "+f"(d[0]), "+f"(d[1]), "+f"(d[2]), "+f"(d[3]), "+f"(d[4]), "+f"(d[5]), "+f"(d[6]), "+f"(d[7]), "+f"(d[8]), "+f"(d[9]), "+f"(d[10]), "+f"(d[11]), "+f"(d[12]), "+f"(d[13]), "+f"(d[14]), "+f"(d[15]), "+f"(d[16]), "+f"(d[17]), "+f"(d[18]), "+f"(d[19]), "+f"(d[20]), "+f"(d[21]), "+f"(d[22]), "+f"(d[23]), "+f"(d[24]), "+f"(d[25]), "+f"(d[26]), "+f"(d[27]), "+f"(d[28]), "+f"(d[29]), "+f"(d[30]), "+f"(d[31]), "+f"(d[32]), "+f"(d[33]), "+f"(d[34]), "+f"(d[35]), "+f"(d[36]), "+f"(d[37]), "+f"(d[38]), "+f"(d[39]), "+f"(d[40]), "+f"(d[41]), "+f"(d[42]), "+f"(d[43]), "+f"(d[44]), "+f"(d[45]), "+f"(d[46]), "+f"(d[47]), "+f"(d[48]), "+f"(d[49]), "+f"(d[50]), "+f"(d[51]), "+f"(d[52]), "+f"(d[53]), "+f"(d[54]), "+f"(d[55]), "+f"(d[56]), "+f"(d[57]), "+f"(d[58]), "+f"(d[59]), "+f"(d[60]), "+f"(d[61]), "+f"(d[62]), "+f"(d[63])
        : "l"(da), "l"(db), "r"(1));
}
__device__ __forceinline__ void wgmma_e5m2_n256(float* d, uint64_t da, uint64_t db) {
    asm volatile(
        "{\n\t.reg .pred p;\n\tsetp.ne.b32 p, %130, 0;\n\t"
        "wgmma.mma_async.sync.aligned.m64n256k32.f32.e5m2.e5m2 "
        "{%0, %1, %2, %3, %4, %5, %6, %7, %8, %9, %10, %11, %12, %13, %14, %15, %16, %17, %18, %19, %20, %21, %22, %23, %24, %25, %26, %27, %28, %29, %30, %31, %32, %33, %34, %35, %36, %37, %38, %39, %40, %41, %42, %43, %44, %45, %46, %47, %48, %49, %50, %51, %52, %53, %54, %55, %56, %57, %58, %59, %60, %61, %62, %63, %64, %65, %66, %67, %68, %69, %70, %71, %72, %73, %74, %75, %76, %77, %78, %79, %80, %81, %82, %83, %84, %85, %86, %87, %88, %89, %90, %91, %92, %93, %94, %95, %96, %97, %98, %99, %100, %101, %102, %103, %104, %105, %106, %107, %108, %109, %110, %111, %112, %113, %114, %115, %116, %117, %118, %119, %120, %121, %122, %123, %124, %125, %126, %127}, %128, %129, p, 1, 1;\n\t}\n"
        : "+f"(d[0]), "+f"(d[1]), "+f"(d[2]), "+f"(d[3]), "+f"(d[4]), "+f"(d[5]), "+f"(d[6]), "+f"(d[7]), "+f"(d[8]), "+f"(d[9]), "+f"(d[10]), "+f"(d[11]), "+f"(d[12]), "+f"(d[13]), "+f"(d[14]), "+f"(d[15]), "+f"(d[16]), "+f"(d[17]), "+f"(d[18]), "+f"(d[19]), "+f"(d[20]), "+f"(d[21]), "+f"(d[22]), "+f"(d[23]), "+f"(d[24]), "+f"(d[25]), "+f"(d[26]), "+f"(d[27]), "+f"(d[28]), "+f"(d[29]), "+f"(d[30]), "+f"(d[31]), "+f"(d[32]), "+f"(d[33]), "+f"(d[34]), "+f"(d[35]), "+f"(d[36]), "+f"(d[37]), "+f"(d[38]), "+f"(d[39]), "+f"(d[40]), "+f"(d[41]), "+f"(d[42]), "+f"(d[43]), "+f"(d[44]), "+f"(d[45]), "+f"(d[46]), "+f"(d[47]), "+f"(d[48]), "+f"(d[49]), "+f"(d[50]), "+f"(d[51]), "+f"(d[52]), "+f"(d[53]), "+f"(d[54]), "+f"(d[55]), "+f"(d[56]), "+f"(d[57]), "+f"(d[58]), "+f"(d[59]), "+f"(d[60]), "+f"(d[61]), "+f"(d[62]), "+f"(d[63]), "+f"(d[64]), "+f"(d[65]), "+f"(d[66]), "+f"(d[67]), "+f"(d[68]), "+f"(d[69]), "+f"(d[70]), "+f"(d[71]), "+f"(d[72]), "+f"(d[73]), "+f"(d[74]), "+f"(d[75]), "+f"(d[76]), "+f"(d[77]), "+f"(d[78]), "+f"(d[79]), "+f"(d[80]), "+f"(d[81]), "+f"(d[82]), "+f"(d[83]), "+f"(d[84]), "+f"(d[85]), "+f"(d[86]), "+f"(d[87]), "+f"(d[88]), "+f"(d[89]), "+f"(d[90]), "+f"(d[91]), "+f"(d[92]), "+f"(d[93]), "+f"(d[94]), "+f"(d[95]), "+f"(d[96]), "+f"(d[97]), "+f"(d[98]), "+f"(d[99]), "+f"(d[100]), "+f"(d[101]), "+f"(d[102]), "+f"(d[103]), "+f"(d[104]), "+f"(d[105]), "+f"(d[106]), "+f"(d[107]), "+f"(d[108]), "+f"(d[109]), "+f"(d[110]), "+f"(d[111]), "+f"(d[112]), "+f"(d[113]), "+f"(d[114]), "+f"(d[115]), "+f"(d[116]), "+f"(d[117]), "+f"(d[118]), "+f"(d[119]), "+f"(d[120]), "+f"(d[121]), "+f"(d[122]), "+f"(d[123]), "+f"(d[124]), "+f"(d[125]), "+f"(d[126]), "+f"(d[127])
        : "l"(da), "l"(db), "r"(1));
}
template <int N>
__device__ __forceinline__ void setmaxnreg_dec() { asm volatile("setmaxnreg.dec.sync.aligned.u32 %0;" ::"n"(N)); }
template <int N>
__device__ __forceinline__ void setmaxnreg_inc() { asm volatile("setmaxnreg.inc.sync.aligned.u32 %0;" ::"n"(N)); }


__device__ __forceinline__ void cp_async_16(void* smem_dst, const void* gmem_src) {
    asm volatile("cp.async.cg.shared.global [%0], [%1], 16;" ::"r"(smem_u32(smem_dst)), "l"(gmem_src) : "memory");
}
__device__ __forceinline__ void cp_async_commit() { asm volatile("cp.async.commit_group;" ::: "memory"); }
template <int N>
__device__ __forceinline__ void cp_async_wait() { asm volatile("cp.async.wait_group %0;" ::"n"(N) : "memory"); }

__device__ __forceinline__ void red_add_v2(float* addr, float a, float b) {
    asm volatile("red.global.add.v2.f32 [%0], {%1, %2};" ::"l"(addr), "f"(a), "f"(b) : "memory");
}
__device__ __forceinline__ void red_add_v4(float* addr, float a, float b, float c, float d) {
    asm volatile("red.global.add.v4.f32 [%0], {%1, %2, %3, %4};" ::"l"(addr), "f"(a), "f"(b),
                 "f"(c), "f"(d)
                 : "memory");
}

__device__ __forceinline__ void red_add_v4_if(bool ok, float* addr, float a, float b, float c, float d) {
    asm volatile(
        "{\n\t"
        ".reg .pred p;\n\t"
        "setp.ne.b32 p, %5, 0;\n\t"
        "@p red.global.add.v4.f32 [%0], {%1, %2, %3, %4};\n\t"
        "}\n" ::"l"(addr), "f"(a), "f"(b), "f"(c), "f"(d), "r"((int)ok)
        : "memory");
}

}
}
```

### pixie_b200/csrc/unet.cu

```cuda
#include "unet.cuh"
#include "conv3d_igemm.cuh"
#include "unet_kernels.cuh"
#include "workspace.cuh"

#include <cmath>
#include <cstdio>
#include <cstdlib>
#include <cstring>
#include <functional>
#include <map>
#include <memory>
#include <string>
#include <vector>

namespace pixie {

namespace {

struct HostTensor {
    std::vector<float> data;
    std::vector<int64_t> shape;
};

struct ConvOp {
    ConvDesc desc;
    ConvPlan plan;
};

struct DevT {
    float* p = nullptr;
    int C = 0, sp = 0;
    double* stats = nullptr;
};

}

}

struct pixie_unet_s {
    pixie_unet_config cfg{};
    std::map<std::string, pixie::HostTensor> params;
    bool finalized = false;
    int NBmax = 1;

    std::vector<void*> allocs;
    std::vector<std::function<int(cudaStream_t)>> ops;
    std::vector<int> op_kinds;
    std::vector<double> op_flops;
    std::vector<std::unique_ptr<pixie::ConvOp>> convs;
    std::map<std::string, pixie::DevT> named;
    int* d_err = nullptr;
    volatile int* h_err = nullptr;
    double* d_stats = nullptr;
    size_t stats_doubles = 0, stats_cap = 0;
    int cur_nb = 1;
    double flops = 0;
    int n_launch = 0;
    pixie::ConvOp* first_conv = nullptr;
    pixie::ConvOp* head_conv = nullptr;
    int feat_cpad = 0;
    __half* feat_staging = nullptr;
    float* out_staging = nullptr;
    struct GraphEntry { cudaGraphExec_t exec = nullptr; const void* feat = nullptr; float* out = nullptr; int nb = 0; };
    static constexpr int kGraphSlots = 4;
    GraphEntry graphs[kGraphSlots];
    int graph_next = 0;
    bool use_graph = true;

    ~pixie_unet_s() {
        for (auto& g : graphs) if (g.exec) cudaGraphExecDestroy(g.exec);
        for (auto& c : convs) pixie::conv_plan_destroy(c->plan);
        for (void* p : allocs) cudaFree(p);
        if (h_err) cudaFreeHost(const_cast<int*>(h_err));
    }
};

namespace pixie {

namespace {

struct Builder {
    UNet& u;
    int NB;
    bool precise;
    bool f8corr;
    bool ok = true;

    explicit Builder(UNet& un) : u(un), NB(un.NBmax), precise(un.cfg.precision >= 1), f8corr(un.cfg.precision == 2) {}

    bool fail(const std::string& m) { if (ok) pixie::fail(m); return ok = false; }
    bool fail(const char* what, cudaError_t e) { if (ok) pixie::fail(what, e); else cudaGetLastError(); return ok = false; }

    template <typename T>
    T* dalloc(size_t n) {
        void* p = nullptr;
        if (const cudaError_t e = cudaMalloc(&p, n * sizeof(T))) { fail("unet_finalize: cudaMalloc", e); return nullptr; }
        u.allocs.push_back(p);
        if (const cudaError_t e = cudaMemset(p, 0, n * sizeof(T))) fail("unet_finalize: cudaMemset", e);
        return reinterpret_cast<T*>(p);
    }
    float* upload(const std::vector<float>& v) {
        float* d = dalloc<float>(v.size());
        if (!d) return nullptr;
        if (const cudaError_t e = cudaMemcpy(d, v.data(), v.size() * 4, cudaMemcpyHostToDevice)) fail("unet_finalize: cudaMemcpy", e);
        return d;
    }
    const HostTensor* param(const std::string& name, size_t expect_numel) {
        auto it = u.params.find(name);
        if (it == u.params.end()) { fail("missing state-dict entry: " + name); return nullptr; }
        if (it->second.data.size() != expect_numel) {
            fail("state-dict entry " + name + " has wrong size");
            return nullptr;
        }
        return &it->second;
    }
    size_t vox(int sp) const { return (size_t)sp * sp * sp; }

    double* stats_slot(int C) {
        double* s = u.d_stats + u.stats_doubles;
        u.stats_doubles += (size_t)NB * C * 2;
        return s;
    }

    struct F16 { __half* hi = nullptr; __half* lo = nullptr; int C = 0; int sp = 0; };

    F16 alloc_f16(int C, int sp) {
        F16 t; t.C = C; t.sp = sp;
        t.hi = dalloc<__half>((size_t)NB * vox(sp) * C);
        if (precise) t.lo = dalloc<__half>((size_t)NB * vox(sp) * C);
        return t;
    }

    void emit_moments(const DevT& x, double* stats) {
        UNet* up = &u;
        const int V = (int)vox(x.sp), C = x.C;
        const float* xp = x.p;
        u.ops.push_back([=](cudaStream_t st) { return launch_moments(xp, up->cur_nb, V, C, stats, st); });
        u.op_kinds.push_back(PIXIE_OP_MOMENTS); u.op_flops.push_back(0);
    }

    void emit_norm(const DevT& x, const double* stats, int mode, int groups, const float* gamma, const float* beta,
                   int act, const F16* dst, int c0, const F16* raw, int raw_c0) {
        NormArgs a;
        a.x = x.p; a.V = (int)vox(x.sp); a.C = x.C; a.stats = stats; a.mode = mode; a.groups = groups;

        a.gamma = gamma; a.beta = beta; a.eps = 1e-5f; a.act = act;
        a.lo_mode = f8corr ? 1 : 0;
        if (dst) { a.dst = dst->hi; a.dst_lo = dst->lo; a.dst_ld = dst->C; a.dst_c0 = c0; }
        if (raw) { a.raw_dst = raw->hi; a.raw_lo = raw->lo; a.raw_ld = raw->C; a.raw_c0 = raw_c0; }
        UNet* up = &u;
        u.ops.push_back([=](cudaStream_t st) { return launch_norm_act(a, up->cur_nb, st); });
        u.op_kinds.push_back(PIXIE_OP_NORM); u.op_flops.push_back(0);
    }

    struct ConvIn { F16 t; int ks; int cin_real; std::string wname; };

    ConvOp* emit_conv(const std::vector<ConvIn>& ins, int sp_out, int stride, int Cout, const float* residual,
                      float* out, bool planar, const std::vector<std::string>& bias_names, DevT* want_stats = nullptr) {
        if (!ok) return nullptr;
        auto op = std::make_unique<ConvOp>();
        const double flops_before = u.flops;
        ConvDesc& d = op->desc;
        d.NB = NB; d.D = d.H = d.W = sp_out; d.stride = stride; d.Cout = Cout;
        d.Cout_pad = (Cout + 15) / 16 * 16;
        d.split_k = 0;
        std::vector<const float*> wptr;
        std::vector<int> cin_real;
        std::vector<std::vector<float>> keep;
        for (const auto& in : ins) {
            const int ks = in.ks, kv = ks * ks * ks;
            const HostTensor* w = param(in.wname, (size_t)Cout * in.cin_real * kv);
            if (!w) return nullptr;
            const int si = (int)d.srcs.size();
            d.srcs.push_back({in.t.hi, in.t.C, in.t.sp, in.t.sp, in.t.sp});
            d.segs.push_back({si, ks, 0});
            wptr.push_back(w->data.data()); cin_real.push_back(in.cin_real);
            u.flops += 2.0 * (double)vox(sp_out) * Cout * in.cin_real * kv;
            if (f8corr && in.t.lo) {
                const int sl = (int)d.srcs.size();
                d.srcs.push_back({in.t.lo, in.t.C, in.t.sp, in.t.sp, in.t.sp});
                ConvDesc::Seg q{sl, ks, 0, 1};
                d.segs.push_back(q);
                wptr.push_back(w->data.data()); cin_real.push_back(in.cin_real);
            } else if (precise && in.t.lo) {
                const int sl = (int)d.srcs.size();
                d.srcs.push_back({in.t.lo, in.t.C, in.t.sp, in.t.sp, in.t.sp});
                d.segs.push_back({sl, ks, 0, 0, 1});
                wptr.push_back(w->data.data()); cin_real.push_back(in.cin_real);
                d.segs.push_back({si, ks, 1});
                wptr.push_back(w->data.data()); cin_real.push_back(in.cin_real);
            } else if (precise) {
                d.segs.push_back({si, ks, 1});
                wptr.push_back(w->data.data()); cin_real.push_back(in.cin_real);
            }
        }
        std::vector<__half> packed;
        conv_pack_weights(d, wptr, cin_real, packed);
        __half* dw = dalloc<__half>(packed.size());
        if (!dw) return nullptr;
        if (const cudaError_t e = cudaMemcpy(dw, packed.data(), packed.size() * 2, cudaMemcpyHostToDevice)) {
            fail("unet_finalize: cudaMemcpy", e);
            return nullptr;
        }
        d.weights = dw;
        std::vector<float> bias(Cout, 0.f);
        for (const auto& bn : bias_names) {
            const HostTensor* b = param(bn, (size_t)Cout);
            if (!b) return nullptr;
            for (int i = 0; i < Cout; ++i) bias[i] += b->data[i];
        }
        d.bias = upload(bias);
        d.residual = residual;
        d.out = out; d.out_ld = Cout; d.out_c0 = 0; d.out_planar = planar ? 1 : 0;
        if (want_stats) { want_stats->stats = stats_slot(Cout); d.stats = want_stats->stats; }
        char e[256] = {0};
        if (conv_plan_create(d, u.d_err, op->plan, e, sizeof(e))) {
            cudaGetLastError();
            fail(e);
            return nullptr;
        }
        ConvOp* raw = op.get();
        UNet* up = &u;
        u.ops.push_back([=](cudaStream_t st) { return conv_plan_launch(raw->plan, up->cur_nb, st); });
        u.op_kinds.push_back(PIXIE_OP_CONV); u.op_flops.push_back(u.flops - flops_before);
        const bool fused = raw->plan.fused_stats;
        u.convs.push_back(std::move(op));
        if (want_stats && !fused) emit_moments(*want_stats, want_stats->stats);
        return raw;
    }

    DevT alloc_f32(int C, int sp, const std::string& name) {
        DevT t; t.C = C; t.sp = sp;
        t.p = dalloc<float>((size_t)NB * vox(sp) * C);
        if (!name.empty()) u.named[name] = t;
        return t;
    }

    DevT resblock(const std::vector<DevT>& xs, int Cout, const std::string& path) {
        const int sp = xs[0].sp;
        int Cin = 0;
        for (auto& x : xs) Cin += x.C;
        const bool has_skip = (Cin != Cout);
        const size_t V = vox(sp);
        const HostTensor* g1 = param(path + ".in_layers.0.weight", V);
        const HostTensor* b1 = param(path + ".in_layers.0.bias", V);
        const HostTensor* g2 = param(path + ".out_layers.0.weight", V);
        const HostTensor* b2 = param(path + ".out_layers.0.bias", V);
        if (!g1 || !b1 || !g2 || !b2) return {};
        const float *dg1 = upload(g1->data), *db1 = upload(b1->data), *dg2 = upload(g2->data), *db2 = upload(b2->data);

        F16 a = alloc_f16(Cin, sp);
        F16 raw;
        if (has_skip) raw = alloc_f16(Cin, sp);
        int c0 = 0;
        for (auto& x : xs) {
            if (!x.stats) { fail("internal: input of " + path + " has no statistics"); return {}; }
            emit_norm(x, x.stats, kNormLN, 1, dg1, db1, kActLeaky, &a, c0, has_skip ? &raw : nullptr, c0);
            c0 += x.C;
        }
        DevT t = alloc_f32(Cout, sp, "");
        if (!emit_conv({{a, 3, Cin, path + ".in_layers.2.weight"}}, sp, 1, Cout, nullptr, t.p, false,
                       {path + ".in_layers.2.bias"}, &t)) return {};
        F16 b = alloc_f16(Cout, sp);
        emit_norm(t, t.stats, kNormLN, 1, dg2, db2, kActLeaky, &b, 0, nullptr, 0);
        DevT out = alloc_f32(Cout, sp, path);
        std::vector<ConvIn> ins = {{b, 3, Cout, path + ".out_layers.3.weight"}};
        std::vector<std::string> biases = {path + ".out_layers.3.bias"};
        if (has_skip) {
            ins.push_back({raw, 1, Cin, path + ".skip_connection.weight"});
            biases.push_back(path + ".skip_connection.bias");
        }
        if (!emit_conv(ins, sp, 1, Cout, has_skip ? nullptr : xs[0].p, out.p, false, biases, &out)) return {};
        u.named[path] = out;
        return out;
    }

    DevT downsample(const DevT& x, const std::string& path) {
        F16 raw = alloc_f16(x.C, x.sp);
        emit_norm(x, nullptr, kNormNone, 1, nullptr, nullptr, kActNone, nullptr, 0, &raw, 0);
        const int sp_out = (x.sp + 1) / 2;
        DevT out = alloc_f32(x.C, sp_out, path);
        if (!emit_conv({{raw, 3, x.C, path + ".op.weight"}}, sp_out, 2, x.C, nullptr, out.p, false, {path + ".op.bias"}, &out)) return {};
        return out;
    }

    DevT upsample(const DevT& x, const std::string& path) {
        F16 up = alloc_f16(x.C, 2 * x.sp);
        {
            UNet* upn = &u;
            const float* xp = x.p; __half* hi = up.hi; __half* lo = up.lo; const int sp = x.sp, C = x.C;
            const int lom = f8corr ? 1 : 0;
            u.ops.push_back([=](cudaStream_t st) { return launch_upsample2(xp, hi, lo, lom, upn->cur_nb, sp, C, st); });
            u.op_kinds.push_back(PIXIE_OP_UPSAMPLE); u.op_flops.push_back(0);
        }
        DevT out = alloc_f32(x.C, 2 * x.sp, path);
        if (!emit_conv({{up, 3, x.C, path + ".conv.weight"}}, 2 * x.sp, 1, x.C, nullptr, out.p, false, {path + ".conv.bias"}, &out)) return {};
        return out;
    }

    DevT attention(const DevT& x, const std::string& path) {
        const int C = x.C, T = (int)vox(x.sp);
        const HostTensor* g = param(path + ".norm.weight", (size_t)C);
        const HostTensor* b = param(path + ".norm.bias", (size_t)C);
        if (!g || !b) return {};
        F16 n = alloc_f16(C, x.sp);
        if (!x.stats) { fail("internal: attention input has no statistics"); return {}; }
        emit_norm(x, x.stats, kNormGN, 32, upload(g->data), upload(b->data), kActNone, &n, 0, nullptr, 0);
        DevT qkv = alloc_f32(3 * C, x.sp, "");
        if (!emit_conv({{n, 1, C, path + ".qkv.weight"}}, x.sp, 1, 3 * C, nullptr, qkv.p, false, {path + ".qkv.bias"})) return {};
        F16 at = alloc_f16(C, x.sp);
        {
            UNet* upn = &u;
            const float* qp = qkv.p; __half* hi = at.hi; __half* lo = at.lo;
            const int lom = f8corr ? 1 : 0;
            u.ops.push_back([=](cudaStream_t s) { return launch_attention(qp, hi, lo, lom, upn->cur_nb, T, C, s); });
            u.op_kinds.push_back(PIXIE_OP_ATTENTION); u.op_flops.push_back(0);
        }
        DevT out = alloc_f32(C, x.sp, path);
        if (!emit_conv({{at, 1, C, path + ".proj_out.weight"}}, x.sp, 1, C, x.p, out.p, false, {path + ".proj_out.bias"}, &out)) return {};
        return out;
    }

    bool build() {
        const pixie_unet_config& c = u.cfg;
        const int G = c.grid_size;
        {
            int* h = nullptr;
            if (const cudaError_t e = cudaHostAlloc(&h, sizeof(int), cudaHostAllocMapped)) return fail("unet_finalize: cudaHostAlloc", e);
            *h = 0;
            u.h_err = h;
            if (const cudaError_t e = cudaHostGetDevicePointer(&u.d_err, h, 0)) return fail("unet_finalize: cudaHostGetDevicePointer", e);
        }
        u.stats_cap = (size_t)NB * 2 * 64 * 1024;
        u.d_stats = dalloc<double>(u.stats_cap);

        u.feat_cpad = (c.feature_channels + 63) / 64 * 64;
        u.feat_staging = dalloc<__half>((size_t)NB * vox(G) * u.feat_cpad);
        F16 feat; feat.hi = u.feat_staging; feat.lo = nullptr; feat.C = u.feat_cpad; feat.sp = G;

        F16 unet_in;
        size_t first_conv_idx = u.convs.size();
        if (c.feature_channels == c.cond_dim) {
            unet_in = feat;
        } else if (c.feature_channels > c.cond_dim) {
            const int Hc = 128;
            DevT c0 = alloc_f32(Hc, G, "projector.net.0");
            if (!emit_conv({{feat, 1, c.feature_channels, "projector.net.0.weight"}}, G, 1, Hc, nullptr, c0.p, false, {"projector.net.0.bias"}, &c0)) return false;
            const HostTensor *g1 = param("projector.net.1.weight", Hc), *b1 = param("projector.net.1.bias", Hc);
            if (!g1 || !b1) return false;
            F16 a1 = alloc_f16(Hc, G);
            emit_norm(c0, c0.stats, kNormGN, 32, upload(g1->data), upload(b1->data), kActSiLU, &a1, 0, nullptr, 0);
            DevT c1 = alloc_f32(Hc, G, "projector.net.3");
            if (!emit_conv({{a1, 3, Hc, "projector.net.3.weight"}}, G, 1, Hc, nullptr, c1.p, false, {"projector.net.3.bias"}, &c1)) return false;
            const HostTensor *g2 = param("projector.net.4.weight", Hc), *b2 = param("projector.net.4.bias", Hc);
            if (!g2 || !b2) return false;
            F16 a2 = alloc_f16(Hc, G);
            emit_norm(c1, c1.stats, kNormGN, 32, upload(g2->data), upload(b2->data), kActSiLU, &a2, 0, nullptr, 0);
            DevT c2 = alloc_f32(c.cond_dim, G, "projector.net.6");
            if (!emit_conv({{a2, 1, Hc, "projector.net.6.weight"}}, G, 1, c.cond_dim, nullptr, c2.p, false, {"projector.net.6.bias"}, &c2)) return false;
            const HostTensor *g3 = param("projector.net.7.weight", c.cond_dim), *b3 = param("projector.net.7.bias", c.cond_dim);
            if (!g3 || !b3) return false;
            unet_in = alloc_f16((c.cond_dim + 63) / 64 * 64, G);
            emit_norm(c2, c2.stats, kNormGN, 32, upload(g3->data), upload(b3->data), kActNone, &unet_in, 0, nullptr, 0);
        } else {
            DevT c0 = alloc_f32(c.cond_dim, G, "projector.net.0");
            if (!emit_conv({{feat, 1, c.feature_channels, "projector.net.0.weight"}}, G, 1, c.cond_dim, nullptr, c0.p, false, {"projector.net.0.bias"}, &c0)) return false;
            const HostTensor *g1 = param("projector.net.1.weight", c.cond_dim), *b1 = param("projector.net.1.bias", c.cond_dim);
            if (!g1 || !b1) return false;
            unet_in = alloc_f16((c.cond_dim + 63) / 64 * 64, G);
            const int groups = c.cond_dim / 2 > 1 ? c.cond_dim / 2 : 1;
            emit_norm(c0, c0.stats, kNormGN, groups, upload(g1->data), upload(b1->data), kActSiLU, &unet_in, 0, nullptr, 0);
        }

        const int mc = c.model_channels;
        std::vector<DevT> hs;
        DevT h = alloc_f32(mc, G, "unet.input_blocks.0");
        if (!emit_conv({{unet_in, 3, c.cond_dim, "unet.input_blocks.0.0.weight"}}, G, 1, mc, nullptr, h.p, false, {"unet.input_blocks.0.0.bias"}, &h)) return false;
        u.first_conv = u.convs[first_conv_idx].get();
        hs.push_back(h);
        int ch = mc, sp = G, blk = 1;
        for (int level = 0; level < c.n_levels; ++level) {
            const int mult = c.channel_mult[level];
            for (int r = 0; r < c.num_res_blocks; ++r) {
                h = resblock({h}, mult * mc, "unet.input_blocks." + std::to_string(blk) + ".0");
                if (!h.p) return false;
                ch = mult * mc;
                hs.push_back(h);
                ++blk;
            }
            if (level != c.n_levels - 1) {
                h = downsample(h, "unet.input_blocks." + std::to_string(blk) + ".0");
                if (!h.p) return false;
                hs.push_back(h);
                ++blk;
                sp = (sp + 1) / 2;
            }
        }
        h = resblock({h}, ch, "unet.middle_block.0");
        if (!h.p) return false;
        h = attention(h, "unet.middle_block.1");
        if (!h.p) return false;
        h = resblock({h}, ch, "unet.middle_block.2");
        if (!h.p) return false;
        int ob = 0;
        for (int level = c.n_levels - 1; level >= 0; --level) {
            const int mult = c.channel_mult[level];
            for (int i = 0; i < c.num_res_blocks + 1; ++i) {
                DevT skip = hs.back();
                hs.pop_back();
                if (skip.sp != h.sp) return fail("odd grid sizes are not supported (crop path :925-930)");
                h = resblock({h, skip}, mc * mult, "unet.output_blocks." + std::to_string(ob) + ".0");
                if (!h.p) return false;
                if (level && i == c.num_res_blocks) {
                    h = upsample(h, "unet.output_blocks." + std::to_string(ob) + ".1");
                    if (!h.p) return false;
                }
                ++ob;
            }
        }
        {
            const size_t V = vox(G);
            const HostTensor *g = param("unet.out.0.weight", V), *b = param("unet.out.0.bias", V);
            if (!g || !b) return false;
            F16 a = alloc_f16(mc, G);
            if (!h.stats) return fail("internal: head input has no statistics");
            emit_norm(h, h.stats, kNormLN, 1, upload(g->data), upload(b->data), kActLeaky, &a, 0, nullptr, 0);
            u.out_staging = dalloc<float>((size_t)NB * c.out_channels * V);
            u.head_conv = emit_conv({{a, 3, mc, "unet.out.2.weight"}}, G, 1, c.out_channels, nullptr, u.out_staging, true, {"unet.out.2.bias"});
            if (!u.head_conv) return false;
        }
        if (u.stats_doubles > u.stats_cap) return fail("stats arena overflow");
        if (!ok) return false;
        const cudaError_t e = cudaDeviceSynchronize();
        return e == cudaSuccess || fail("unet_finalize", e);
    }
};

}

UNet* unet_create(const pixie_unet_config& cfg) {
    if (cfg.n_levels < 1 || cfg.n_levels > 8) { fail("n_levels out of range"); return nullptr; }
    if (cfg.grid_size % (1 << (cfg.n_levels - 1))) { fail("grid_size must be divisible by 2^(levels-1)"); return nullptr; }
    if (cfg.model_channels % 64) { fail("model_channels must be a multiple of 64"); return nullptr; }
    if (cfg.precision < 0 || cfg.precision > 2) { fail("precision must be 0 (fp16), 1 (fp16x3) or 2 (fp16 + e5m2 corrections)"); return nullptr; }
    auto* u = new UNet();
    u->cfg = cfg;
    u->use_graph = getenv("PIXIE_NO_GRAPH") == nullptr;
    u->NBmax = cfg.max_batch > 0 ? cfg.max_batch : 1;
    return u;
}

int unet_set_tensor(UNet* u, const char* name, const float* data, const int64_t* shape, int ndim) {
    if (u->finalized) return fail("set_tensor after finalize");
    HostTensor t;
    size_t n = 1;
    for (int i = 0; i < ndim; ++i) { t.shape.push_back(shape[i]); n *= (size_t)shape[i]; }
    t.data.assign(data, data + n);
    u->params[name] = std::move(t);
    return 0;
}

int unet_finalize(UNet* u) {
    if (u->finalized) return 0;
    Builder b(*u);
    if (!b.build()) return 1;
    u->params.clear();
    u->finalized = true;
    u->n_launch = (int)u->ops.size() + 1;
    return 0;
}

static int enqueue_ops(UNet* u, cudaStream_t st) {
    if (const cudaError_t e = cudaMemsetAsync(u->d_stats, 0, u->stats_doubles * sizeof(double), st)) return fail("unet_forward: statistics clear", e);
    for (auto& op : u->ops)
        if (const int rc = op(st)) return fail("unet_forward: kernel launch", (cudaError_t)rc);
    return 0;
}

static int run_ops(UNet* u, int batch, const void* feat, float* out, cudaStream_t st) {
    u->cur_nb = batch;
    if (u->use_graph) {
        UNet::GraphEntry* hit = nullptr;
        for (auto& g : u->graphs) if (g.exec && g.nb == batch && g.feat == feat && g.out == out) hit = &g;
        if (!hit) {
            UNet::GraphEntry& slot = u->graphs[u->graph_next];
            u->graph_next = (u->graph_next + 1) % UNet::kGraphSlots;
            if (slot.exec) { cudaGraphExecDestroy(slot.exec); slot.exec = nullptr; }
            cudaStream_t cs = nullptr;
            cudaGraph_t g = nullptr;
            bool ok = cudaStreamCreateWithFlags(&cs, cudaStreamNonBlocking) == cudaSuccess &&
                      cudaStreamBeginCapture(cs, cudaStreamCaptureModeThreadLocal) == cudaSuccess;
            if (ok) {
                const int rc = enqueue_ops(u, cs);
                ok = (cudaStreamEndCapture(cs, &g) == cudaSuccess) && g && rc == 0;
            }
            if (ok) ok = cudaGraphInstantiate(&slot.exec, g, 0) == cudaSuccess;
            if (g) cudaGraphDestroy(g);
            if (cs) cudaStreamDestroy(cs);
            if (!ok) { cudaGetLastError(); slot.exec = nullptr; u->use_graph = false; }
            else { slot.nb = batch; slot.feat = feat; slot.out = out; hit = &slot; }
        }
        if (hit && hit->exec) {
            const cudaError_t e = cudaGraphLaunch(hit->exec, st);
            return e == cudaSuccess ? 0 : fail("unet_forward: cudaGraphLaunch", e);
        }
    }
    return enqueue_ops(u, st);
}

static int check_err_flag(UNet* u) {
    const int h = u->h_err ? *u->h_err : 0;
    if (h) {
        *u->h_err = 0;
        return fail("conv pipeline timeout (device flag " + std::to_string(h) + "): the outputs of the affected forward are invalid");
    }
    return 0;
}

int unet_forward(UNet* u, const void* feat_f16, int batch, float* out, cudaStream_t st) {
    if (!u->finalized) return fail("forward before finalize");
    if (check_err_flag(u)) return 1;
    if (batch < 1 || batch > u->NBmax) return fail("batch exceeds max_batch");
    ConvOp* fc = u->first_conv;
    const __half* fp = reinterpret_cast<const __half*>(feat_f16);
    char e[256] = {0};
    if (fc->desc.srcs[0].ptr != fp) {
        fc->desc.srcs[0].ptr = fp;
        if (conv_plan_retarget(fc->desc, fc->plan, e, sizeof(e))) return fail(e);
    }
    u->head_conv->plan.p.out = out;
    return run_ops(u, batch, feat_f16, out, st);
}

static cudaError_t time_ops(UNet* u, int batch, cudaStream_t st, std::vector<cudaEvent_t>& ev, float* ms) {
    for (auto& e : ev) PIXIE_TRY(cudaEventCreate(&e));
    u->cur_nb = batch;
    PIXIE_TRY(cudaMemsetAsync(u->d_stats, 0, u->stats_doubles * sizeof(double), st));
    PIXIE_TRY(cudaEventRecord(ev[0], st));
    for (size_t i = 0; i < u->ops.size(); ++i) {
        PIXIE_TRY((cudaError_t)u->ops[i](st));
        PIXIE_TRY(cudaEventRecord(ev[i + 1], st));
    }
    PIXIE_TRY(cudaStreamSynchronize(st));
    for (size_t i = 0; i < u->ops.size(); ++i) PIXIE_TRY(cudaEventElapsedTime(&ms[i], ev[i], ev[i + 1]));
    return cudaSuccess;
}

int unet_profile(UNet* u, const void* feat_f16, int batch, float* out, cudaStream_t st, float* ms, int* kinds, double* flops, int cap) {
    if (!u->finalized) { fail("profile before finalize"); return -1; }
    const int n = (int)u->ops.size();
    if (cap < n) { fail("profile: buffers too small"); return -1; }
    if (unet_forward(u, feat_f16, batch, out, st)) return -1;
    std::vector<cudaEvent_t> ev(n + 1, nullptr);
    const cudaError_t e = time_ops(u, batch, st, ev, ms);
    for (cudaEvent_t x : ev) if (x) cudaEventDestroy(x);
    if (e != cudaSuccess) { fail("unet_profile", e); return -1; }
    for (int i = 0; i < n; ++i) {
        kinds[i] = u->op_kinds[i];
        flops[i] = u->op_flops[i];
    }
    return n;
}

int unet_forward_ncdhw(UNet* u, const float* feat_f32, int batch, float* out, cudaStream_t st) {
    if (!u->finalized) return fail("forward before finalize");
    if (batch < 1 || batch > u->NBmax) return fail("batch exceeds max_batch");
    const long long V = (long long)u->cfg.grid_size * u->cfg.grid_size * u->cfg.grid_size;
    if (const int rc = launch_ncdhw_to_ndhwc_f16(feat_f32, u->feat_staging, batch, u->cfg.feature_channels, u->feat_cpad, V, st))
        return fail("unet_forward_ncdhw: layout conversion", (cudaError_t)rc);
    return unet_forward(u, u->feat_staging, batch, out, st);
}

int unet_forward_host(UNet* u, const void* feat_host, int batch, float* out_host, cudaStream_t st) {
    if (!u->finalized) return fail("forward before finalize");
    if (batch < 1 || batch > u->NBmax) return fail("batch exceeds max_batch");
    if (u->feat_cpad != u->cfg.feature_channels) return fail("forward_host needs feature_channels % 64 == 0");
    const size_t V = (size_t)u->cfg.grid_size * u->cfg.grid_size * u->cfg.grid_size;
    if (const cudaError_t e = cudaMemcpyAsync(u->feat_staging, feat_host, (size_t)batch * V * u->feat_cpad * 2, cudaMemcpyHostToDevice, st))
        return fail("unet_forward_host: host-to-device copy", e);
    if (unet_forward(u, u->feat_staging, batch, u->out_staging, st)) return 1;
    if (const cudaError_t e = cudaMemcpyAsync(out_host, u->out_staging, (size_t)batch * u->cfg.out_channels * V * 4, cudaMemcpyDeviceToHost, st))
        return fail("unet_forward_host: device-to-host copy", e);
    if (const cudaError_t e = cudaStreamSynchronize(st)) return fail("unet_forward_host", e);
    return check_err_flag(u);
}

int64_t unet_debug_fetch(UNet* u, const char* name, float* host_out, int64_t capacity) {
    auto it = u->named.find(name);
    if (it == u->named.end()) { fail(std::string("no such activation: ") + name); return -1; }
    const DevT& t = it->second;
    const int64_t n = (int64_t)u->cur_nb * t.sp * t.sp * t.sp * t.C;
    if (n > capacity) { fail("debug_fetch: buffer too small"); return -2; }
    if (const cudaError_t e = cudaDeviceSynchronize()) { fail("unet_debug_fetch", e); return -3; }
    if (check_err_flag(u)) return -4;
    if (const cudaError_t e = cudaMemcpy(host_out, t.p, (size_t)n * 4, cudaMemcpyDeviceToHost)) { fail("unet_debug_fetch", e); return -3; }
    return n;
}

std::string unet_debug_names(UNet* u) {
    std::string s;
    for (const auto& kv : u->named)
        s += kv.first + " " + std::to_string(kv.second.C) + " " + std::to_string(kv.second.sp) + "\n";
    return s;
}

int unet_launch_count(UNet* u) {
    int n = 1;
    for (auto& c : u->convs) n += c->plan.needs_zero ? 1 : 0;
    return n + (int)u->ops.size();
}
double unet_flops(UNet* u) { return u->flops; }
int unet_check(UNet* u) {
    if (const cudaError_t e = cudaDeviceSynchronize()) return fail("unet_check", e);
    return check_err_flag(u);
}
void unet_destroy(UNet* u) { delete u; }

}
```

### pixie_b200/csrc/unet_kernels.cu

```cuda
#include "unet_kernels.cuh"

#include <cuda_fp16.h>
#include <cuda_fp8.h>
#include <cstdint>
#include <cstdlib>

#include "conv3d_igemm.cuh"

namespace pixie {

namespace {

__device__ __forceinline__ float act_apply(float v, int act) {
    if (act == kActLeaky) return v > 0.f ? v : 0.02f * v;
    if (act == kActSiLU) return __fdividef(v, 1.f + __expf(-v));
    return v;
}

__device__ __forceinline__ uint32_t pack_e5m2x4(float a, float b, float c, float d) {
    const uint32_t lo = __nv_cvt_float2_to_fp8x2(make_float2(a, b), __NV_SATFINITE, __NV_E5M2);
    const uint32_t hi = __nv_cvt_float2_to_fp8x2(make_float2(c, d), __NV_SATFINITE, __NV_E5M2);
    return lo | (hi << 16);
}

template <int LOM>
__device__ __forceinline__ void store_hi_lo_t(const float (&f)[4], __half* hi, __half* lo, size_t idx, int lo_mode) {
    if (LOM == 2) lo = nullptr;
    if (LOM == 0 || LOM == 1) lo_mode = LOM;
    __half2 r0 = __floats2half2_rn(f[0], f[1]), r1 = __floats2half2_rn(f[2], f[3]);
    uint2 pk; pk.x = *reinterpret_cast<uint32_t*>(&r0); pk.y = *reinterpret_cast<uint32_t*>(&r1);
    *reinterpret_cast<uint2*>(hi + idx) = pk;
    if (lo && lo_mode == 1) {
        const float2 b0 = __half22float2(r0), b1 = __half22float2(r1);
        constexpr float up = (float)(1 << kF8Shift), down = 1.0f / (float)(1 << kF8Shift);
        uint8_t* row = reinterpret_cast<uint8_t*>(lo) + 2 * (idx & ~(size_t)63) + (idx & 63);
        *reinterpret_cast<uint32_t*>(row) = pack_e5m2x4((f[0] - b0.x) * up, (f[1] - b0.y) * up, (f[2] - b1.x) * up, (f[3] - b1.y) * up);
        *reinterpret_cast<uint32_t*>(row + 64) = pack_e5m2x4(f[0] * down, f[1] * down, f[2] * down, f[3] * down);
    } else if (lo) {
        const float2 b0 = __half22float2(r0), b1 = __half22float2(r1);
        __half2 l0 = __floats2half2_rn(f[0] - b0.x, f[1] - b0.y), l1 = __floats2half2_rn(f[2] - b1.x, f[3] - b1.y);
        uint2 pl; pl.x = *reinterpret_cast<uint32_t*>(&l0); pl.y = *reinterpret_cast<uint32_t*>(&l1);
        *reinterpret_cast<uint2*>(lo + idx) = pl;
    }
}
__device__ __forceinline__ void store_hi_lo(const float (&f)[4], __half* hi, __half* lo, size_t idx, int lo_mode) {
    store_hi_lo_t<-1>(f, hi, lo, idx, lo_mode);
}

}

__global__ void __launch_bounds__(256)
moments_kernel(const float* __restrict__ x, int V, int C, int vox_per_block, double* __restrict__ stats) {
    const int cols4 = C >> 2;
    const int rows_par = 256 / cols4;
    const int col = threadIdx.x % cols4;
    const int row = threadIdx.x / cols4;
    const int nb = blockIdx.y;
    const int v0 = blockIdx.x * vox_per_block;
    const int v1 = min(V, v0 + vox_per_block);
    float s[4] = {0, 0, 0, 0}, q[4] = {0, 0, 0, 0};
    const float4* xp = reinterpret_cast<const float4*>(x + ((size_t)nb * V) * C) + col;
    const float4 pv = __ldg(xp);
    const float p[4] = {pv.x, pv.y, pv.z, pv.w};
    if (row < rows_par) {
#pragma unroll 4
        for (int v = v0 + row; v < v1; v += rows_par) {
            const float4 a = __ldg(xp + (size_t)v * cols4);
            const float d[4] = {a.x - p[0], a.y - p[1], a.z - p[2], a.w - p[3]};
#pragma unroll
            for (int j = 0; j < 4; ++j) { s[j] += d[j]; q[j] = fmaf(d[j], d[j], q[j]); }
        }
    }
    __shared__ float sh[256 * 8];
    float* mine = sh + threadIdx.x * 8;
#pragma unroll
    for (int j = 0; j < 4; ++j) { mine[j] = s[j]; mine[4 + j] = q[j]; }
    __syncthreads();
    if (threadIdx.x < cols4) {
        double ds[4] = {0, 0, 0, 0}, dq[4] = {0, 0, 0, 0};
        for (int r = 0; r < rows_par; ++r) {
            const float* o = sh + (r * cols4 + threadIdx.x) * 8;
#pragma unroll
            for (int j = 0; j < 4; ++j) { ds[j] += o[j]; dq[j] += o[4 + j]; }
        }
        double* st = stats + ((size_t)nb * C + threadIdx.x * 4) * 2;
        const double n = (double)max(0, v1 - v0);
#pragma unroll
        for (int j = 0; j < 4; ++j) {
            const double pj = p[j];
            atomicAdd(st + 2 * j, ds[j] + n * pj);
            atomicAdd(st + 2 * j + 1, dq[j] + pj * (2.0 * ds[j] + n * pj));
        }
    }
}

template <int MODE, int ACT, int LOM>
__global__ void __launch_bounds__(256)
norm_act_kernel(NormArgs a) {
    __shared__ float s_mean[1024], s_rstd[1024], s_g[1024], s_b[1024];
    const int nb = blockIdx.y;
    if (MODE != kNormNone) {
        const int cg = (MODE == kNormGN) ? a.C / a.groups : 1;
        for (int ch = threadIdx.x; ch < a.C; ch += blockDim.x) {
            const int grp0 = (ch / cg) * cg;
            double s = 0, q = 0;
            for (int k = 0; k < cg; ++k) {
                s += a.stats[((size_t)nb * a.C + grp0 + k) * 2];
                q += a.stats[((size_t)nb * a.C + grp0 + k) * 2 + 1];
            }
            const double n = (double)a.V * cg;
            const double m = s / n;
            double var = q / n - m * m;
            if (var < 0) var = 0;
            s_mean[ch] = (float)m;
            s_rstd[ch] = (float)(1.0 / sqrt(var + (double)a.eps));
            s_g[ch] = (MODE == kNormGN) ? a.gamma[ch] : 1.f;
            s_b[ch] = (MODE == kNormGN) ? a.beta[ch] : 0.f;
        }
        __syncthreads();
    }
    const int cols4 = a.C >> 2;
    const int rows_par = 256 / cols4;
    const int col = threadIdx.x % cols4;
    const int row = threadIdx.x / cols4;
    if (row >= rows_par) return;
    const int c = col * 4;
    float mean[4] = {0, 0, 0, 0}, rstd[4] = {1, 1, 1, 1}, g[4] = {1, 1, 1, 1}, b[4] = {0, 0, 0, 0};
    if (MODE != kNormNone) {
#pragma unroll
        for (int j = 0; j < 4; ++j) { mean[j] = s_mean[c + j]; rstd[j] = s_rstd[c + j]; g[j] = s_g[c + j]; b[j] = s_b[c + j]; }
    }
    const int v0 = blockIdx.x * a.vox_per_block;
    const int v1 = min(a.V, v0 + a.vox_per_block);
    const float4* xp = reinterpret_cast<const float4*>(a.x + ((size_t)nb * a.V) * a.C) + col;
    constexpr int U = 4;
    for (int vb = v0 + row; vb < v1; vb += rows_par * U) {
        float4 xv[U];
        float gv[U], bv[U];
#pragma unroll
        for (int u = 0; u < U; ++u) {
            const int v = vb + u * rows_par;
            const bool in = v < v1;
            xv[u] = in ? __ldg(xp + (size_t)v * cols4) : make_float4(0.f, 0.f, 0.f, 0.f);
            gv[u] = 1.f; bv[u] = 0.f;
            if (in && MODE == kNormLN && a.dst) { gv[u] = __ldg(a.gamma + v); bv[u] = __ldg(a.beta + v); }
        }
#pragma unroll
        for (int u = 0; u < U; ++u) {
            const int v = vb + u * rows_par;
            if (v >= v1) break;
            float f[4] = {xv[u].x, xv[u].y, xv[u].z, xv[u].w};
            if (a.raw_dst) store_hi_lo_t<-1>(f, a.raw_dst, a.raw_lo, ((size_t)nb * a.V + v) * a.raw_ld + a.raw_c0 + c, a.lo_mode);
            if (a.dst) {
#pragma unroll
                for (int j = 0; j < 4; ++j) {
                    float y = f[j];
                    if (MODE == kNormLN) y = (y - mean[j]) * rstd[j] * gv[u] + bv[u];
                    else if (MODE == kNormGN) y = (y - mean[j]) * rstd[j] * g[j] + b[j];
                    f[j] = act_apply(y, ACT);
                }
                store_hi_lo_t<LOM>(f, a.dst, a.dst_lo, ((size_t)nb * a.V + v) * a.dst_ld + a.dst_c0 + c, a.lo_mode);
            }
        }
    }
}

__global__ void __launch_bounds__(256)
upsample2_kernel(const float* __restrict__ x, __half* __restrict__ y, __half* __restrict__ ylo, int lo_mode, int sp, int C, long long total4) {
    const long long i = (long long)blockIdx.x * blockDim.x + threadIdx.x;
    if (i >= total4) return;
    const int cols4 = C >> 2;
    const int col = (int)(i % cols4);
    long long v = i / cols4;
    const int S = 2 * sp;
    const int w = (int)(v % S); v /= S;
    const int h = (int)(v % S); v /= S;
    const int d = (int)(v % S); v /= S;
    const long long nb = v;
    const long long src = ((nb * sp + (d >> 1)) * sp + (h >> 1)) * sp + (w >> 1);
    const float4 a = __ldg(reinterpret_cast<const float4*>(x + src * C) + col);
    const float f[4] = {a.x, a.y, a.z, a.w};
    store_hi_lo(f, y, ylo, (size_t)i * 4, lo_mode);
}

constexpr int kAttnQ = 4;
__global__ void __launch_bounds__(256)
attention_kernel(const float* __restrict__ qkv, __half* __restrict__ out, __half* __restrict__ out_lo, int lo_mode, int T, int C) {
    extern __shared__ __align__(16) float sm[];
    float* qs = sm;
    float* sc = sm + kAttnQ * C;
    __shared__ float inv_s[kAttnQ];
    const int t0 = blockIdx.x * kAttnQ, nb = blockIdx.y;
    const int warp = threadIdx.x >> 5, lane = threadIdx.x & 31, nwarp = blockDim.x >> 5;
    const float* base = qkv + (size_t)nb * T * 3 * C;
    const float scale = rsqrtf(sqrtf((float)C));
    for (int i = threadIdx.x; i < kAttnQ * C; i += blockDim.x) {
        const int q = i / C, c = i - q * C;
        qs[i] = (t0 + q < T) ? base[(size_t)(t0 + q) * 3 * C + c] * scale : 0.f;
    }
    __syncthreads();
    for (int s = warp; s < T; s += nwarp) {
        const float4* kp = reinterpret_cast<const float4*>(base + (size_t)s * 3 * C + C);
        float part[kAttnQ];
#pragma unroll
        for (int q = 0; q < kAttnQ; ++q) part[q] = 0.f;
        for (int c4 = lane; c4 < C / 4; c4 += 32) {
            float4 kv = __ldg(kp + c4);
            kv.x *= scale; kv.y *= scale; kv.z *= scale; kv.w *= scale;
#pragma unroll
            for (int q = 0; q < kAttnQ; ++q) {
                const float4 qv = *reinterpret_cast<const float4*>(qs + q * C + 4 * c4);
                part[q] += qv.x * kv.x + qv.y * kv.y + qv.z * kv.z + qv.w * kv.w;
            }
        }
#pragma unroll
        for (int q = 0; q < kAttnQ; ++q) {
            float v = part[q];
            for (int o = 16; o; o >>= 1) v += __shfl_xor_sync(0xffffffffu, v, o);
            if (lane == 0) sc[q * T + s] = v;
        }
    }
    __syncthreads();
    if (warp < kAttnQ) {
        float* row = sc + warp * T;
        float mx = -INFINITY;
        for (int s = lane; s < T; s += 32) mx = fmaxf(mx, row[s]);
        for (int o = 16; o; o >>= 1) mx = fmaxf(mx, __shfl_xor_sync(0xffffffffu, mx, o));
        float sum = 0.f;
        for (int s = lane; s < T; s += 32) { const float e = __expf(row[s] - mx); row[s] = e; sum += e; }
        for (int o = 16; o; o >>= 1) sum += __shfl_xor_sync(0xffffffffu, sum, o);
        if (lane == 0) inv_s[warp] = 1.f / sum;
    }
    __syncthreads();
    for (int c = threadIdx.x; c < C; c += blockDim.x) {
        float acc[kAttnQ];
#pragma unroll
        for (int q = 0; q < kAttnQ; ++q) acc[q] = 0.f;
        const float* vp = base + 2 * C + c;
#pragma unroll 4
        for (int s = 0; s < T; ++s) {
            const float v = __ldg(vp + (size_t)s * 3 * C);
#pragma unroll
            for (int q = 0; q < kAttnQ; ++q) acc[q] = fmaf(sc[q * T + s], v, acc[q]);
        }
#pragma unroll
        for (int q = 0; q < kAttnQ; ++q) {
            if (t0 + q >= T) break;
            const float val = acc[q] * inv_s[q];
            const __half hv = __float2half_rn(val);
            const size_t idx = ((size_t)nb * T + t0 + q) * C + c;
            out[idx] = hv;
            if (out_lo && lo_mode == 1) {
                constexpr float up = (float)(1 << kF8Shift), down = 1.0f / (float)(1 << kF8Shift);
                uint8_t* row = reinterpret_cast<uint8_t*>(out_lo) + 2 * (idx & ~(size_t)63) + (idx & 63);
                row[0] = (uint8_t)__nv_cvt_float_to_fp8((val - __half2float(hv)) * up, __NV_SATFINITE, __NV_E5M2);
                row[64] = (uint8_t)__nv_cvt_float_to_fp8(val * down, __NV_SATFINITE, __NV_E5M2);
            } else if (out_lo) out_lo[idx] = __float2half_rn(val - __half2float(hv));
        }
    }
}

__global__ void __launch_bounds__(256)
ncdhw_to_ndhwc_f16_kernel(const float* __restrict__ x, __half* __restrict__ y, int C, int Cpad, long long V) {
    const long long i = (long long)blockIdx.x * blockDim.x + threadIdx.x;
    const int nb = blockIdx.y;
    if (i >= V * Cpad) return;
    const int c = (int)(i % Cpad);
    const long long v = i / Cpad;
    const float val = c < C ? x[((size_t)nb * C + c) * V + v] : 0.f;
    y[(size_t)nb * V * Cpad + i] = __float2half_rn(val);
}

__global__ void __launch_bounds__(256)
pack_predictions_kernel(const float* __restrict__ seg, const float* __restrict__ cont, float* __restrict__ out,
                        long long V, int n_classes) {
    const long long v = (long long)blockIdx.x * blockDim.x + threadIdx.x;
    const int nb = blockIdx.y;
    if (v >= V) return;
    const float* sp = seg + (size_t)nb * n_classes * V;
    int best = 0;
    float bv = sp[v];
    for (int c = 1; c < n_classes; ++c) {
        const float x = sp[(size_t)c * V + v];
        if (x > bv) { bv = x; best = c; }
    }
    float* op = out + (size_t)nb * (3 + n_classes) * V;
    for (int c = 0; c < 3; ++c) op[(size_t)c * V + v] = cont[((size_t)nb * 3 + c) * V + v];
    for (int c = 0; c < n_classes; ++c) op[(size_t)(3 + c) * V + v] = (c == best) ? 1.f : 0.f;
}

int launch_pack_predictions(const float* seg, const float* cont, float* out, int NB, long long V, int n_classes, cudaStream_t st) {
    dim3 grid((unsigned)((V + 255) / 256), NB);
    pack_predictions_kernel<<<grid, 256, 0, st>>>(seg, cont, out, V, n_classes);
    return (int)cudaGetLastError();
}

template <typename K>
static inline void prefer_max_smem_carveout(K kernel) {
    static const bool on = !(getenv("PIXIE_UNET_CARVEOUT") && atoi(getenv("PIXIE_UNET_CARVEOUT")) == 0);
    if (on) cudaFuncSetAttribute(kernel, cudaFuncAttributePreferredSharedMemoryCarveout, (int)cudaSharedmemCarveoutMaxShared);
}
#define PIXIE_CARVEOUT_ONCE(kernel) do { static bool done_ = false; if (!done_) { prefer_max_smem_carveout(kernel); done_ = true; } } while (0)

static inline int vox_per_block_for(int V, int C) {
    const int trip = (256 / (C / 4)) * 4;
    int vpb = (V + 295) / 296;
    vpb = (vpb + trip - 1) / trip * trip;
    return vpb < trip ? trip : (vpb > 512 ? 512 : vpb);
}

int launch_moments(const float* x, int NB, int V, int C, double* stats, cudaStream_t st) {
    if (C % 4 || C / 4 > 256) return 1;
    const int vpb = vox_per_block_for(V, C);
    dim3 grid((V + vpb - 1) / vpb, NB);
    PIXIE_CARVEOUT_ONCE(moments_kernel);
    moments_kernel<<<grid, 256, 0, st>>>(x, V, C, vpb, stats);
    return (int)cudaGetLastError();
}

int launch_norm_act(NormArgs a, int NB, cudaStream_t st) {
    if (a.C % 4 || a.C / 4 > 256) return 1;
    a.vox_per_block = vox_per_block_for(a.V, a.C);
    dim3 grid((a.V + a.vox_per_block - 1) / a.vox_per_block, NB);
    const int lom = !a.dst_lo ? 2 : (a.lo_mode == 1 ? 1 : 0);
#define PIXIE_NORM_L(M, A) \
    do { if (lom == 2) { PIXIE_CARVEOUT_ONCE((norm_act_kernel<M, A, 2>)); norm_act_kernel<M, A, 2><<<grid, 256, 0, st>>>(a); } \
         else if (lom == 1) { PIXIE_CARVEOUT_ONCE((norm_act_kernel<M, A, 1>)); norm_act_kernel<M, A, 1><<<grid, 256, 0, st>>>(a); } \
         else { PIXIE_CARVEOUT_ONCE((norm_act_kernel<M, A, 0>)); norm_act_kernel<M, A, 0><<<grid, 256, 0, st>>>(a); } } while (0)
#define PIXIE_NORM_A(M) \
    do { if (a.act == kActSiLU) PIXIE_NORM_L(M, kActSiLU); else if (a.act == kActLeaky) PIXIE_NORM_L(M, kActLeaky); else PIXIE_NORM_L(M, kActNone); } while (0)
    if (a.mode == kNormLN) PIXIE_NORM_A(kNormLN);
    else if (a.mode == kNormGN) PIXIE_NORM_A(kNormGN);
    else PIXIE_NORM_A(kNormNone);
#undef PIXIE_NORM_A
#undef PIXIE_NORM_L
    return (int)cudaGetLastError();
}

int launch_upsample2(const float* x, __half* y, __half* ylo, int lo_mode, int NB, int sp, int C, cudaStream_t st) {
    const long long total4 = (long long)NB * 8 * sp * sp * sp * (C / 4);
    PIXIE_CARVEOUT_ONCE(upsample2_kernel);
    upsample2_kernel<<<(unsigned)((total4 + 255) / 256), 256, 0, st>>>(x, y, ylo, lo_mode, sp, C, total4);
    return (int)cudaGetLastError();
}

int launch_attention(const float* qkv, __half* out, __half* out_lo, int lo_mode, int NB, int T, int C, cudaStream_t st) {
    const size_t smem = (size_t)kAttnQ * (C + T) * sizeof(float);
    if (smem > 48 * 1024 || C % 4) return 1;
    dim3 grid((T + kAttnQ - 1) / kAttnQ, NB);
    PIXIE_CARVEOUT_ONCE(attention_kernel);
    attention_kernel<<<grid, 256, smem, st>>>(qkv, out, out_lo, lo_mode, T, C);
    return (int)cudaGetLastError();
}

int launch_ncdhw_to_ndhwc_f16(const float* x, __half* y, int NB, int C, int Cpad, long long V, cudaStream_t st) {
    dim3 grid((unsigned)((V * Cpad + 255) / 256), NB);
    ncdhw_to_ndhwc_f16_kernel<<<grid, 256, 0, st>>>(x, y, C, Cpad, V);
    return (int)cudaGetLastError();
}

}
```

### pixie_b200/csrc/unet_kernels.cuh

```cuda
#pragma once
#include <cuda_runtime.h>
#include <cuda_fp16.h>

namespace pixie {

enum { kNormNone = 0, kNormLN = 1, kNormGN = 2 };
enum { kActNone = 0, kActLeaky = 1, kActSiLU = 2 };

struct NormArgs {
    const float* x = nullptr;
    int V = 0, C = 0;
    const double* stats = nullptr;
    int mode = kNormNone;
    int groups = 1;
    const float* gamma = nullptr;
    const float* beta = nullptr;
    float eps = 1e-5f;
    int act = kActNone;
    __half* dst = nullptr;
    __half* dst_lo = nullptr;
    int lo_mode = 0;
    int dst_ld = 0, dst_c0 = 0;
    __half* raw_dst = nullptr;
    __half* raw_lo = nullptr;
    int raw_ld = 0, raw_c0 = 0;
    int vox_per_block = 0;
};

int launch_moments(const float* x, int NB, int V, int C, double* stats, cudaStream_t st);
int launch_norm_act(NormArgs a, int NB, cudaStream_t st);
int launch_upsample2(const float* x, __half* y, __half* ylo, int lo_mode, int NB, int sp, int C, cudaStream_t st);
int launch_attention(const float* qkv, __half* out, __half* out_lo, int lo_mode, int NB, int T, int C, cudaStream_t st);
int launch_pack_predictions(const float* seg, const float* cont, float* out, int NB, long long V, int n_classes, cudaStream_t st);
int launch_ncdhw_to_ndhwc_f16(const float* x, __half* y, int NB, int C, int Cpad, long long V, cudaStream_t st);

}
```

Baseline: 16.17 million.

## Use serial split-K fixup workspace and programmatic dependent launch across U-Net ops

Split-K conv outputs now go to a per-tile workspace, and a counter picks the last-arriving CTA to reduce the partials and run the full epilogue. This replaces atomic/red adds into a memset-zeroed output and lets split-K convs keep fused stats. Every U-Net kernel is also launched through cudaLaunchKernelEx with programmatic stream serialization and calls griddepcontrol.wait, so its prologue can overlap the previous kernel's tail. The cost is extra workspace traffic, a counter atomic per tile and the risk of ordering bugs.

```diff
diff --git a/pixie_b200/csrc/capi.cu b/pixie_b200/csrc/capi.cu
--- a/pixie_b200/csrc/capi.cu
+++ b/pixie_b200/csrc/capi.cu
@@ -279,7 +279,8 @@
     if (!seg_logits_dev || !cont_dev || !out_dev) return fail("null argument");
     if (require_device()) return 1;
     return check("pack_predictions",
-                 (cudaError_t)pixie::launch_pack_predictions(seg_logits_dev, cont_dev, out_dev, batch, voxels, n_classes, (cudaStream_t)stream));
+                 (cudaError_t)pixie::launch_pack_predictions(seg_logits_dev, cont_dev, out_dev, batch, voxels, n_classes, (cudaStream_t)stream,
+                                                             true));
 }
 int pixie_unet_launch_count(pixie_unet_t h) { return h ? pixie::unet_launch_count(h) : 0; }
 double pixie_unet_flops(pixie_unet_t h) { return h ? pixie::unet_flops(h) : 0.0; }
diff --git a/pixie_b200/csrc/conv3d_igemm.cu b/pixie_b200/csrc/conv3d_igemm.cu
--- a/pixie_b200/csrc/conv3d_igemm.cu
+++ b/pixie_b200/csrc/conv3d_igemm.cu
@@ -25,6 +25,7 @@
     uint64_t sfull[kMaxSStages];
     uint64_t sempty[kMaxSStages];
     int abort_flag;
+    int splitk_last;
 };
 
 constexpr int kCtlBarrierBytes = 512;
@@ -191,7 +192,53 @@
     if (p.stats != nullptr && !p.stats_scalar)
         for (int i = threadIdx.x; i < 2 * p.stats_ld; i += n_threads) m.stats[i] = 0.f;
     __syncthreads();
+    pdl_wait();
     return m;
+}
+
+template <int NREG>
+__device__ __forceinline__ bool splitk_fixup(const ConvKernelParams& p, int wi, int split, float* acc, SmemCtrl* ctl) {
+    static_assert(NREG % 4 == 0, "accumulators move as float4");
+    constexpr int N4 = NREG / 4;
+    const unsigned tile = (unsigned)wi / (unsigned)p.split_k;
+    float4* slots = reinterpret_cast<float4*>(p.splitk_ws) + (size_t)tile * p.split_k * N4 * 256 + threadIdx.x;
+    float4* mine = slots + (size_t)split * N4 * 256;
+#pragma unroll
+    for (int i = 0; i < N4; ++i) __stcg(mine + (size_t)i * 256, make_float4(acc[4 * i], acc[4 * i + 1], acc[4 * i + 2], acc[4 * i + 3]));
+    __threadfence();
+    asm volatile("bar.sync 1, 256;" ::: "memory");
+    if (threadIdx.x == 0) {
+        const bool last = atomicAdd(p.splitk_cnt + tile, 1u) == (unsigned)p.split_k - 1;
+        if (last) p.splitk_cnt[tile] = 0u;
+        ctl->splitk_last = last ? 1 : 0;
+    }
+    asm volatile("bar.sync 1, 256;" ::: "memory");
+    if (!ctl->splitk_last) return false;
+    __threadfence();
+    constexpr int C4 = N4 < 4 ? N4 : 4, kU = 4;
+#pragma unroll
+    for (int j = 0; j < NREG; ++j) acc[j] = 0.f;
+#pragma unroll
+    for (int i0 = 0; i0 < N4; i0 += C4) {
+        for (int s0 = 0; s0 < p.split_k; s0 += kU) {
+            float4 v[kU][C4];
+#pragma unroll
+            for (int u = 0; u < kU; ++u)
+#pragma unroll
+                for (int i = 0; i < C4; ++i)
+                    v[u][i] = s0 + u < p.split_k ? __ldcg(slots + ((size_t)(s0 + u) * N4 + i0 + i) * 256) : make_float4(0.f, 0.f, 0.f, 0.f);
+#pragma unroll
+            for (int u = 0; u < kU; ++u) {
+                if (s0 + u >= p.split_k) break;
+#pragma unroll
+                for (int i = 0; i < C4; ++i) {
+                    float* a = acc + 4 * (i0 + i);
+                    a[0] += v[u][i].x; a[1] += v[u][i].y; a[2] += v[u][i].z; a[3] += v[u][i].w;
+                }
+            }
+        }
+    }
+    return true;
 }
 
 __device__ __forceinline__ void conv_report_abort(const ConvKernelParams& p, const SmemCtrl* ctl) {
@@ -336,11 +383,11 @@
 #pragma unroll
                 for (int j = 0; j < BN / 2; ++j) fence_operand(acc[d][j]);
             if (!ok) break;
+            if (p.split_k > 1 && !splitk_fixup<TD * BN / 2>(p, wi, t.split, &acc[0][0], ctl)) continue;
 
             if (do_stats) stats.enter(p, t.nb, lane);
-            const bool first_split = (t.split == 0);
-            const bool use_bias = first_split && p.bias != nullptr;
-            const bool use_res = first_split && p.residual != nullptr;
+            const bool use_bias = p.bias != nullptr;
+            const bool use_res = p.residual != nullptr;
 #pragma unroll
             for (int d = 0; d < TD; ++d) {
                 if (d >= t.tde) break;
@@ -364,11 +411,11 @@
                             const long long i0 = ((long long)t.nb * p.Cout + ch) * DHW + vox;
                             if (ok0) {
                                 if (use_res) v0 += p.residual[i0];
-                                if (p.atomic_out) atomicAdd(p.out + i0, v0); else p.out[i0] = v0;
+                                p.out[i0] = v0;
                             }
                             if (ok1) {
                                 if (use_res) v1 += p.residual[i0 + DHW];
-                                if (p.atomic_out) atomicAdd(p.out + i0 + DHW, v1); else p.out[i0 + DHW] = v1;
+                                p.out[i0 + DHW] = v1;
                             }
                         } else if (ok0) {
                             const long long base = ((long long)t.nb * DHW + vox) * p.out_ld + p.out_c0 + ch;
@@ -377,12 +424,11 @@
                                     const float2 rv = __ldg(reinterpret_cast<const float2*>(p.residual + base));
                                     v0 += rv.x; v1 += rv.y;
                                 }
-                                if (p.atomic_out) red_add_v2(p.out + base, v0, v1);
-                                else *reinterpret_cast<float2*>(p.out + base) = make_float2(v0, v1);
+                                *reinterpret_cast<float2*>(p.out + base) = make_float2(v0, v1);
                             } else {
                                 if (use_res) { v0 += p.residual[base]; if (ok1) v1 += p.residual[base + 1]; }
-                                if (p.atomic_out) { atomicAdd(p.out + base, v0); if (ok1) atomicAdd(p.out + base + 1, v1); }
-                                else { p.out[base] = v0; if (ok1) p.out[base + 1] = v1; }
+                                p.out[base] = v0;
+                                if (ok1) p.out[base + 1] = v1;
                             }
                         }
                         a0 = ok0 ? v0 : 0.f;
@@ -512,16 +558,16 @@
 #pragma unroll
             for (int j = 0; j < NV / 2; ++j) fence_operand(acc[j]);
             if (!ok) break;
+            if (p.split_k > 1 && !splitk_fixup<NV / 2>(p, wi, t.split, acc, ctl)) continue;
 
             if (do_stats) stats.enter(p, t.nb, lane);
             if (!has_plane) continue;
-            const bool first_split = (t.split == 0);
             const int ch = t.n0 + 4 * q4;
             const bool ch_ok = ch < p.Cout;
             float4 bias4 = make_float4(0.f, 0.f, 0.f, 0.f);
-            if (first_split && p.bias != nullptr && ch_ok)
+            if (p.bias != nullptr && ch_ok)
                 bias4 = make_float4(__ldg(p.bias + ch), __ldg(p.bias + ch + 1), __ldg(p.bias + ch + 2), __ldg(p.bias + ch + 3));
-            const bool use_res = first_split && p.residual != nullptr;
+            const bool use_res = p.residual != nullptr;
             const long long plane_base = ((long long)t.nb * p.D + t.d0 + g) * p.H;
             float st_s[4] = {0.f, 0.f, 0.f, 0.f}, st_q[4] = {0.f, 0.f, 0.f, 0.f};
 #pragma unroll
@@ -548,8 +594,7 @@
                             const float4 rv = __ldg(reinterpret_cast<const float4*>(p.residual + base));
                             x.x += rv.x; x.y += rv.y; x.z += rv.z; x.w += rv.w;
                         }
-                        if (p.atomic_out) red_add_v4(p.out + base, x.x, x.y, x.z, x.w);
-                        else *reinterpret_cast<float4*>(p.out + base) = x;
+                        *reinterpret_cast<float4*>(p.out + base) = x;
                         st_s[0] += x.x; st_s[1] += x.y; st_s[2] += x.z; st_s[3] += x.w;
                         st_q[0] = fmaf(x.x, x.x, st_q[0]); st_q[1] = fmaf(x.y, x.y, st_q[1]);
                         st_q[2] = fmaf(x.z, x.z, st_q[2]); st_q[3] = fmaf(x.w, x.w, st_q[3]);
@@ -816,6 +861,10 @@
     return true;
 }
 
+static int plan_regs_per_thread(bool channel_major, const ConvKernelParams& p) {
+    return channel_major ? p.TH * p.TW / 2 : p.TD * p.block_n / 2;
+}
+
 int conv_plan_create(const ConvDesc& d, int* d_err_flag, ConvPlan& plan, char* err, int errlen) {
     auto fail = [&](const char* m) { snprintf(err, errlen, "conv_plan_create: %s", m); return 1; };
     PFN_encodeTiled enc = get_encode_fn();
@@ -866,14 +915,12 @@
     split = std::max(1, std::min(split, p.n_phases));
     if ((long long)p.n_phases * (split + 1) >= (1ll << 31)) return fail("too many phases for the split-K bookkeeping");
     p.split_k = split;
-    p.atomic_out = split > 1;
-    plan.needs_zero = split > 1;
 
     for (size_t i = 0; i < slots.size(); ++i) p.slab_rows[i] = p.TW * (p.TH + slots[i].n_kh - 1);
     int max_rows = 0;
     for (size_t i = 0; i < slots.size(); ++i) max_rows = std::max(max_rows, p.slab_rows[i]);
     p.s_stage_bytes = max_rows * 128;
-    plan.fused_stats = d.stats != nullptr && split == 1 && d.Cout <= kStatsMaxC && !d.out_planar;
+    plan.fused_stats = d.stats != nullptr && d.Cout <= kStatsMaxC && !d.out_planar;
     p.stats_ld = (d.Cout + 31) / 32 * 32;
     const int stats_bytes = plan.fused_stats ? 2 * p.stats_ld * 4 : 0;
     const int ctl_core = kCtlBarrierBytes + (plan.channel_major ? 2 * kCmStageFloats * 4 : 0) + stats_bytes;
@@ -911,8 +958,11 @@
     p.err_flag = d_err_flag;
     p.stats = plan.fused_stats ? d.stats : nullptr;
     p.stats_scalar = d.stats_scalar ? 1 : 0;
-    plan.out_item_bytes = d.out_planar ? (size_t)d.Cout * d.D * d.H * d.W * 4
-                                       : (size_t)d.D * d.H * d.W * p.out_ld * 4;
+    if (split > 1) {
+        const int regs = plan_regs_per_thread(plan.channel_major, p);
+        plan.splitk_tiles = items;
+        plan.splitk_ws_floats = (size_t)items * split * regs * 256;
+    }
 
     plan.grid = std::min(items * split, sms);
 
@@ -928,14 +978,22 @@
     plan.d_phases = nullptr;
 }
 
-int conv_plan_launch(const ConvPlan& plan, int nb, cudaStream_t stream) {
+int conv_plan_launch(const ConvPlan& plan, int nb, cudaStream_t stream, bool pdl) {
     if (nb < 1 || nb > plan.p.NB) return (int)cudaErrorInvalidValue;
+    if (plan.p.split_k > 1 && (!plan.p.splitk_ws || !plan.p.splitk_cnt)) return (int)cudaErrorInvalidValue;
     ConvKernelParams p = plan.p;
     p.NB = nb;
-    const int grid = std::min(plan.grid, conv_work_items(nb, p.tiles_d, p.tiles_h, p.tiles_w, p.n_tiles, p.split_k));
-    if (plan.needs_zero) cudaMemsetAsync(p.out, 0, plan.out_item_bytes * (size_t)nb, stream);
-    plan.kernel<<<grid, plan.threads, plan.smem_bytes, stream>>>(p);
-    return (int)cudaGetLastError();
-}
-
-}
+    cudaLaunchConfig_t cfg{};
+    cfg.gridDim = dim3(std::min(plan.grid, conv_work_items(nb, p.tiles_d, p.tiles_h, p.tiles_w, p.n_tiles, p.split_k)));
+    cfg.blockDim = dim3(plan.threads);
+    cfg.dynamicSmemBytes = plan.smem_bytes;
+    cfg.stream = stream;
+    cudaLaunchAttribute attr[1];
+    attr[0].id = cudaLaunchAttributeProgrammaticStreamSerialization;
+    attr[0].val.programmaticStreamSerializationAllowed = 1;
+    cfg.attrs = attr;
+    cfg.numAttrs = pdl ? 1 : 0;
+    return (int)cudaLaunchKernelEx(&cfg, plan.kernel, p);
+}
+
+}
diff --git a/pixie_b200/csrc/conv3d_igemm.cuh b/pixie_b200/csrc/conv3d_igemm.cuh
--- a/pixie_b200/csrc/conv3d_igemm.cuh
+++ b/pixie_b200/csrc/conv3d_igemm.cuh
@@ -39,6 +39,8 @@
     const ConvPhase* phases;
     int n_phases;
     int split_k;
+    float* splitk_ws;
+    unsigned* splitk_cnt;
     int NB, D, H, W;
     int stride;
     int TW, TH, TD;
@@ -55,7 +57,6 @@
     int out_ld;
     int out_c0;
     int out_planar;
-    int atomic_out;
     double* stats;
     int stats_ld;
     int smem_slack;
@@ -108,13 +109,13 @@
     int threads = 0;
     int grid = 0;
     int smem_bytes = 0;
-    bool needs_zero = false;
     bool fused_stats = false;
-    size_t out_item_bytes = 0;
+    size_t splitk_ws_floats = 0;
+    int splitk_tiles = 0;
 };
 
 int conv_plan_create(const ConvDesc& d, int* d_err_flag, ConvPlan& plan, char* err, int errlen);
 void conv_plan_destroy(ConvPlan& plan);
-int conv_plan_launch(const ConvPlan& plan, int nb, cudaStream_t stream);
+int conv_plan_launch(const ConvPlan& plan, int nb, cudaStream_t stream, bool pdl = false);
 int conv_plan_retarget(const ConvDesc& d, ConvPlan& plan, char* err, int errlen);
 }
diff --git a/pixie_b200/csrc/ptx.cuh b/pixie_b200/csrc/ptx.cuh
--- a/pixie_b200/csrc/ptx.cuh
+++ b/pixie_b200/csrc/ptx.cuh
@@ -193,14 +193,7 @@
 template <int N>
 __device__ __forceinline__ void cp_async_wait() { asm volatile("cp.async.wait_group %0;" ::"n"(N) : "memory"); }
 
-__device__ __forceinline__ void red_add_v2(float* addr, float a, float b) {
-    asm volatile("red.global.add.v2.f32 [%0], {%1, %2};" ::"l"(addr), "f"(a), "f"(b) : "memory");
-}
-__device__ __forceinline__ void red_add_v4(float* addr, float a, float b, float c, float d) {
-    asm volatile("red.global.add.v4.f32 [%0], {%1, %2, %3, %4};" ::"l"(addr), "f"(a), "f"(b),
-                 "f"(c), "f"(d)
-                 : "memory");
-}
+__device__ __forceinline__ void pdl_wait() { asm volatile("griddepcontrol.wait;" ::: "memory"); }
 
 __device__ __forceinline__ void red_add_v4_if(bool ok, float* addr, float a, float b, float c, float d) {
     asm volatile(
diff --git a/pixie_b200/csrc/unet.cu b/pixie_b200/csrc/unet.cu
--- a/pixie_b200/csrc/unet.cu
+++ b/pixie_b200/csrc/unet.cu
@@ -3,6 +3,7 @@
 #include "unet_kernels.cuh"
 #include "workspace.cuh"
 
+#include <algorithm>
 #include <cmath>
 #include <cstdio>
 #include <cstdlib>
@@ -44,7 +45,7 @@
     int NBmax = 1;
 
     std::vector<void*> allocs;
-    std::vector<std::function<int(cudaStream_t)>> ops;
+    std::vector<std::function<int(cudaStream_t, bool)>> ops;
     std::vector<int> op_kinds;
     std::vector<double> op_flops;
     std::vector<std::unique_ptr<pixie::ConvOp>> convs;
@@ -53,9 +54,11 @@
     volatile int* h_err = nullptr;
     double* d_stats = nullptr;
     size_t stats_doubles = 0, stats_cap = 0;
+    float* splitk_ws = nullptr;
+    unsigned* splitk_cnt = nullptr;
+    int splitk_tiles = 0;
     int cur_nb = 1;
     double flops = 0;
-    int n_launch = 0;
     pixie::ConvOp* first_conv = nullptr;
     pixie::ConvOp* head_conv = nullptr;
     int feat_cpad = 0;
@@ -135,7 +138,7 @@
         UNet* up = &u;
         const int V = (int)vox(x.sp), C = x.C;
         const float* xp = x.p;
-        u.ops.push_back([=](cudaStream_t st) { return launch_moments(xp, up->cur_nb, V, C, stats, st); });
+        u.ops.push_back([=](cudaStream_t st, bool pdl) { return launch_moments(xp, up->cur_nb, V, C, stats, st, pdl); });
         u.op_kinds.push_back(PIXIE_OP_MOMENTS); u.op_flops.push_back(0);
     }
 
@@ -149,7 +152,7 @@
         if (dst) { a.dst = dst->hi; a.dst_lo = dst->lo; a.dst_ld = dst->C; a.dst_c0 = c0; }
         if (raw) { a.raw_dst = raw->hi; a.raw_lo = raw->lo; a.raw_ld = raw->C; a.raw_c0 = raw_c0; }
         UNet* up = &u;
-        u.ops.push_back([=](cudaStream_t st) { return launch_norm_act(a, up->cur_nb, st); });
+        u.ops.push_back([=](cudaStream_t st, bool pdl) { return launch_norm_act(a, up->cur_nb, st, pdl); });
         u.op_kinds.push_back(PIXIE_OP_NORM); u.op_flops.push_back(0);
     }
 
@@ -221,7 +224,7 @@
         }
         ConvOp* raw = op.get();
         UNet* up = &u;
-        u.ops.push_back([=](cudaStream_t st) { return conv_plan_launch(raw->plan, up->cur_nb, st); });
+        u.ops.push_back([=](cudaStream_t st, bool pdl) { return conv_plan_launch(raw->plan, up->cur_nb, st, pdl); });
         u.op_kinds.push_back(PIXIE_OP_CONV); u.op_flops.push_back(u.flops - flops_before);
         const bool fused = raw->plan.fused_stats;
         u.convs.push_back(std::move(op));
@@ -290,7 +293,7 @@
             UNet* upn = &u;
             const float* xp = x.p; __half* hi = up.hi; __half* lo = up.lo; const int sp = x.sp, C = x.C;
             const int lom = f8corr ? 1 : 0;
-            u.ops.push_back([=](cudaStream_t st) { return launch_upsample2(xp, hi, lo, lom, upn->cur_nb, sp, C, st); });
+            u.ops.push_back([=](cudaStream_t st, bool pdl) { return launch_upsample2(xp, hi, lo, lom, upn->cur_nb, sp, C, st, pdl); });
             u.op_kinds.push_back(PIXIE_OP_UPSAMPLE); u.op_flops.push_back(0);
         }
         DevT out = alloc_f32(x.C, 2 * x.sp, path);
@@ -313,7 +316,7 @@
             UNet* upn = &u;
             const float* qp = qkv.p; __half* hi = at.hi; __half* lo = at.lo;
             const int lom = f8corr ? 1 : 0;
-            u.ops.push_back([=](cudaStream_t s) { return launch_attention(qp, hi, lo, lom, upn->cur_nb, T, C, s); });
+            u.ops.push_back([=](cudaStream_t s, bool pdl) { return launch_attention(qp, hi, lo, lom, upn->cur_nb, T, C, s, pdl); });
             u.op_kinds.push_back(PIXIE_OP_ATTENTION); u.op_flops.push_back(0);
         }
         DevT out = alloc_f32(C, x.sp, path);
@@ -431,6 +434,23 @@
         }
         if (u.stats_doubles > u.stats_cap) return fail("stats arena overflow");
         if (!ok) return false;
+        {
+            size_t ws = 0;
+            for (auto& c : u.convs) {
+                ws = std::max(ws, c->plan.splitk_ws_floats);
+                u.splitk_tiles = std::max(u.splitk_tiles, c->plan.splitk_tiles);
+            }
+            if (ws) {
+                u.splitk_ws = dalloc<float>(ws);
+                u.splitk_cnt = dalloc<unsigned>((size_t)u.splitk_tiles);
+                if (!ok) return false;
+                for (auto& c : u.convs) {
+                    if (c->plan.p.split_k == 1) continue;
+                    c->plan.p.splitk_ws = u.splitk_ws;
+                    c->plan.p.splitk_cnt = u.splitk_cnt;
+                }
+            }
+        }
         const cudaError_t e = cudaDeviceSynchronize();
         return e == cudaSuccess || fail("unet_finalize", e);
     }
@@ -466,14 +486,13 @@
     if (!b.build()) return 1;
     u->params.clear();
     u->finalized = true;
-    u->n_launch = (int)u->ops.size() + 1;
     return 0;
 }
 
 static int enqueue_ops(UNet* u, cudaStream_t st) {
     if (const cudaError_t e = cudaMemsetAsync(u->d_stats, 0, u->stats_doubles * sizeof(double), st)) return fail("unet_forward: statistics clear", e);
-    for (auto& op : u->ops)
-        if (const int rc = op(st)) return fail("unet_forward: kernel launch", (cudaError_t)rc);
+    for (size_t i = 0; i < u->ops.size(); ++i)
+        if (const int rc = u->ops[i](st, i > 0)) return fail("unet_forward: kernel launch", (cudaError_t)rc);
     return 0;
 }
 
@@ -512,6 +531,10 @@
     const int h = u->h_err ? *u->h_err : 0;
     if (h) {
         *u->h_err = 0;
+        if (u->splitk_cnt) {
+            cudaDeviceSynchronize();
+            cudaMemset(u->splitk_cnt, 0, (size_t)u->splitk_tiles * sizeof(unsigned));
+        }
         return fail("conv pipeline timeout (device flag " + std::to_string(h) + "): the outputs of the affected forward are invalid");
     }
     return 0;
@@ -538,7 +561,7 @@
     PIXIE_TRY(cudaMemsetAsync(u->d_stats, 0, u->stats_doubles * sizeof(double), st));
     PIXIE_TRY(cudaEventRecord(ev[0], st));
     for (size_t i = 0; i < u->ops.size(); ++i) {
-        PIXIE_TRY((cudaError_t)u->ops[i](st));
+        PIXIE_TRY((cudaError_t)u->ops[i](st, false));
         PIXIE_TRY(cudaEventRecord(ev[i + 1], st));
     }
     PIXIE_TRY(cudaStreamSynchronize(st));
@@ -566,7 +589,7 @@
     if (!u->finalized) return fail("forward before finalize");
     if (batch < 1 || batch > u->NBmax) return fail("batch exceeds max_batch");
     const long long V = (long long)u->cfg.grid_size * u->cfg.grid_size * u->cfg.grid_size;
-    if (const int rc = launch_ncdhw_to_ndhwc_f16(feat_f32, u->feat_staging, batch, u->cfg.feature_channels, u->feat_cpad, V, st))
+    if (const int rc = launch_ncdhw_to_ndhwc_f16(feat_f32, u->feat_staging, batch, u->cfg.feature_channels, u->feat_cpad, V, st, true))
         return fail("unet_forward_ncdhw: layout conversion", (cudaError_t)rc);
     return unet_forward(u, u->feat_staging, batch, out, st);
 }
@@ -604,11 +627,7 @@
     return s;
 }
 
-int unet_launch_count(UNet* u) {
-    int n = 1;
-    for (auto& c : u->convs) n += c->plan.needs_zero ? 1 : 0;
-    return n + (int)u->ops.size();
-}
+int unet_launch_count(UNet* u) { return 1 + (int)u->ops.size(); }
 double unet_flops(UNet* u) { return u->flops; }
 int unet_check(UNet* u) {
     if (const cudaError_t e = cudaDeviceSynchronize()) return fail("unet_check", e);
diff --git a/pixie_b200/csrc/unet_kernels.cu b/pixie_b200/csrc/unet_kernels.cu
--- a/pixie_b200/csrc/unet_kernels.cu
+++ b/pixie_b200/csrc/unet_kernels.cu
@@ -6,10 +6,13 @@
 #include <cstdlib>
 
 #include "conv3d_igemm.cuh"
+#include "ptx.cuh"
 
 namespace pixie {
 
 namespace {
+
+__device__ __forceinline__ void pdl_enter() { ptx::pdl_wait(); }
 
 __device__ __forceinline__ float act_apply(float v, int act) {
     if (act == kActLeaky) return v > 0.f ? v : 0.02f * v;
@@ -51,6 +54,7 @@
 
 __global__ void __launch_bounds__(256)
 moments_kernel(const float* __restrict__ x, int V, int C, int vox_per_block, double* __restrict__ stats) {
+    pdl_enter();
     const int cols4 = C >> 2;
     const int rows_par = 256 / cols4;
     const int col = threadIdx.x % cols4;
@@ -97,6 +101,7 @@
 template <int MODE, int ACT, int LOM>
 __global__ void __launch_bounds__(256)
 norm_act_kernel(NormArgs a) {
+    pdl_enter();
     __shared__ float s_mean[1024], s_rstd[1024], s_g[1024], s_b[1024];
     const int nb = blockIdx.y;
     if (MODE != kNormNone) {
@@ -167,6 +172,7 @@
 
 __global__ void __launch_bounds__(256)
 upsample2_kernel(const float* __restrict__ x, __half* __restrict__ y, __half* __restrict__ ylo, int lo_mode, int sp, int C, long long total4) {
+    pdl_enter();
     const long long i = (long long)blockIdx.x * blockDim.x + threadIdx.x;
     if (i >= total4) return;
     const int cols4 = C >> 2;
@@ -186,6 +192,7 @@
 constexpr int kAttnQ = 4;
 __global__ void __launch_bounds__(256)
 attention_kernel(const float* __restrict__ qkv, __half* __restrict__ out, __half* __restrict__ out_lo, int lo_mode, int T, int C) {
+    pdl_enter();
     extern __shared__ __align__(16) float sm[];
     float* qs = sm;
     float* sc = sm + kAttnQ * C;
@@ -262,6 +269,7 @@
 
 __global__ void __launch_bounds__(256)
 ncdhw_to_ndhwc_f16_kernel(const float* __restrict__ x, __half* __restrict__ y, int C, int Cpad, long long V) {
+    pdl_enter();
     const long long i = (long long)blockIdx.x * blockDim.x + threadIdx.x;
     const int nb = blockIdx.y;
     if (i >= V * Cpad) return;
@@ -274,6 +282,7 @@
 __global__ void __launch_bounds__(256)
 pack_predictions_kernel(const float* __restrict__ seg, const float* __restrict__ cont, float* __restrict__ out,
                         long long V, int n_classes) {
+    pdl_enter();
     const long long v = (long long)blockIdx.x * blockDim.x + threadIdx.x;
     const int nb = blockIdx.y;
     if (v >= V) return;
@@ -289,10 +298,20 @@
     for (int c = 0; c < n_classes; ++c) op[(size_t)(3 + c) * V + v] = (c == best) ? 1.f : 0.f;
 }
 
-int launch_pack_predictions(const float* seg, const float* cont, float* out, int NB, long long V, int n_classes, cudaStream_t st) {
-    dim3 grid((unsigned)((V + 255) / 256), NB);
-    pack_predictions_kernel<<<grid, 256, 0, st>>>(seg, cont, out, V, n_classes);
-    return (int)cudaGetLastError();
+template <typename... KArgs, typename... Args>
+static int launch_k(void (*kern)(KArgs...), dim3 grid, int smem, cudaStream_t st, bool pdl, Args... args) {
+    cudaLaunchConfig_t cfg{};
+    cfg.gridDim = grid; cfg.blockDim = dim3(256); cfg.dynamicSmemBytes = smem; cfg.stream = st;
+    cudaLaunchAttribute attr[1];
+    attr[0].id = cudaLaunchAttributeProgrammaticStreamSerialization;
+    attr[0].val.programmaticStreamSerializationAllowed = 1;
+    cfg.attrs = attr; cfg.numAttrs = pdl ? 1 : 0;
+    return (int)cudaLaunchKernelEx(&cfg, kern, KArgs(args)...);
+}
+
+int launch_pack_predictions(const float* seg, const float* cont, float* out, int NB, long long V, int n_classes, cudaStream_t st,
+                            bool pdl) {
+    return launch_k(pack_predictions_kernel, dim3((unsigned)((V + 255) / 256), NB), 0, st, pdl, seg, cont, out, V, n_classes);
 }
 
 template <typename K>
@@ -309,24 +328,24 @@
     return vpb < trip ? trip : (vpb > 512 ? 512 : vpb);
 }
 
-int launch_moments(const float* x, int NB, int V, int C, double* stats, cudaStream_t st) {
+int launch_moments(const float* x, int NB, int V, int C, double* stats, cudaStream_t st, bool pdl) {
     if (C % 4 || C / 4 > 256) return 1;
     const int vpb = vox_per_block_for(V, C);
     dim3 grid((V + vpb - 1) / vpb, NB);
     PIXIE_CARVEOUT_ONCE(moments_kernel);
-    moments_kernel<<<grid, 256, 0, st>>>(x, V, C, vpb, stats);
-    return (int)cudaGetLastError();
-}
-
-int launch_norm_act(NormArgs a, int NB, cudaStream_t st) {
+    return launch_k(moments_kernel, grid, 0, st, pdl, x, V, C, vpb, stats);
+}
+
+int launch_norm_act(NormArgs a, int NB, cudaStream_t st, bool pdl) {
     if (a.C % 4 || a.C / 4 > 256) return 1;
     a.vox_per_block = vox_per_block_for(a.V, a.C);
     dim3 grid((a.V + a.vox_per_block - 1) / a.vox_per_block, NB);
     const int lom = !a.dst_lo ? 2 : (a.lo_mode == 1 ? 1 : 0);
+    int rc = 0;
 #define PIXIE_NORM_L(M, A) \
-    do { if (lom == 2) { PIXIE_CARVEOUT_ONCE((norm_act_kernel<M, A, 2>)); norm_act_kernel<M, A, 2><<<grid, 256, 0, st>>>(a); } \
-         else if (lom == 1) { PIXIE_CARVEOUT_ONCE((norm_act_kernel<M, A, 1>)); norm_act_kernel<M, A, 1><<<grid, 256, 0, st>>>(a); } \
-         else { PIXIE_CARVEOUT_ONCE((norm_act_kernel<M, A, 0>)); norm_act_kernel<M, A, 0><<<grid, 256, 0, st>>>(a); } } while (0)
+    do { if (lom == 2) { PIXIE_CARVEOUT_ONCE((norm_act_kernel<M, A, 2>)); rc = launch_k(norm_act_kernel<M, A, 2>, grid, 0, st, pdl, a); } \
+         else if (lom == 1) { PIXIE_CARVEOUT_ONCE((norm_act_kernel<M, A, 1>)); rc = launch_k(norm_act_kernel<M, A, 1>, grid, 0, st, pdl, a); } \
+         else { PIXIE_CARVEOUT_ONCE((norm_act_kernel<M, A, 0>)); rc = launch_k(norm_act_kernel<M, A, 0>, grid, 0, st, pdl, a); } } while (0)
 #define PIXIE_NORM_A(M) \
     do { if (a.act == kActSiLU) PIXIE_NORM_L(M, kActSiLU); else if (a.act == kActLeaky) PIXIE_NORM_L(M, kActLeaky); else PIXIE_NORM_L(M, kActNone); } while (0)
     if (a.mode == kNormLN) PIXIE_NORM_A(kNormLN);
@@ -334,29 +353,26 @@
     else PIXIE_NORM_A(kNormNone);
 #undef PIXIE_NORM_A
 #undef PIXIE_NORM_L
-    return (int)cudaGetLastError();
-}
-
-int launch_upsample2(const float* x, __half* y, __half* ylo, int lo_mode, int NB, int sp, int C, cudaStream_t st) {
+    return rc;
+}
+
+int launch_upsample2(const float* x, __half* y, __half* ylo, int lo_mode, int NB, int sp, int C, cudaStream_t st, bool pdl) {
     const long long total4 = (long long)NB * 8 * sp * sp * sp * (C / 4);
     PIXIE_CARVEOUT_ONCE(upsample2_kernel);
-    upsample2_kernel<<<(unsigned)((total4 + 255) / 256), 256, 0, st>>>(x, y, ylo, lo_mode, sp, C, total4);
-    return (int)cudaGetLastError();
-}
-
-int launch_attention(const float* qkv, __half* out, __half* out_lo, int lo_mode, int NB, int T, int C, cudaStream_t st) {
+    return launch_k(upsample2_kernel, dim3((unsigned)((total4 + 255) / 256)), 0, st, pdl, x, y, ylo, lo_mode, sp, C, total4);
+}
+
+int launch_attention(const float* qkv, __half* out, __half* out_lo, int lo_mode, int NB, int T, int C, cudaStream_t st, bool pdl) {
     const size_t smem = (size_t)kAttnQ * (C + T) * sizeof(float);
     if (smem > 48 * 1024 || C % 4) return 1;
     dim3 grid((T + kAttnQ - 1) / kAttnQ, NB);
     PIXIE_CARVEOUT_ONCE(attention_kernel);
-    attention_kernel<<<grid, 256, smem, st>>>(qkv, out, out_lo, lo_mode, T, C);
-    return (int)cudaGetLastError();
-}
-
-int launch_ncdhw_to_ndhwc_f16(const float* x, __half* y, int NB, int C, int Cpad, long long V, cudaStream_t st) {
+    return launch_k(attention_kernel, grid, (int)smem, st, pdl, qkv, out, out_lo, lo_mode, T, C);
+}
+
+int launch_ncdhw_to_ndhwc_f16(const float* x, __half* y, int NB, int C, int Cpad, long long V, cudaStream_t st, bool pdl) {
     dim3 grid((unsigned)((V * Cpad + 255) / 256), NB);
-    ncdhw_to_ndhwc_f16_kernel<<<grid, 256, 0, st>>>(x, y, C, Cpad, V);
-    return (int)cudaGetLastError();
-}
-
-}
+    return launch_k(ncdhw_to_ndhwc_f16_kernel, grid, 0, st, pdl, x, y, C, Cpad, V);
+}
+
+}
diff --git a/pixie_b200/csrc/unet_kernels.cuh b/pixie_b200/csrc/unet_kernels.cuh
--- a/pixie_b200/csrc/unet_kernels.cuh
+++ b/pixie_b200/csrc/unet_kernels.cuh
@@ -27,11 +27,13 @@
     int vox_per_block = 0;
 };
 
-int launch_moments(const float* x, int NB, int V, int C, double* stats, cudaStream_t st);
-int launch_norm_act(NormArgs a, int NB, cudaStream_t st);
-int launch_upsample2(const float* x, __half* y, __half* ylo, int lo_mode, int NB, int sp, int C, cudaStream_t st);
-int launch_attention(const float* qkv, __half* out, __half* out_lo, int lo_mode, int NB, int T, int C, cudaStream_t st);
-int launch_pack_predictions(const float* seg, const float* cont, float* out, int NB, long long V, int n_classes, cudaStream_t st);
-int launch_ncdhw_to_ndhwc_f16(const float* x, __half* y, int NB, int C, int Cpad, long long V, cudaStream_t st);
+int launch_moments(const float* x, int NB, int V, int C, double* stats, cudaStream_t st, bool pdl = false);
+int launch_norm_act(NormArgs a, int NB, cudaStream_t st, bool pdl = false);
+int launch_upsample2(const float* x, __half* y, __half* ylo, int lo_mode, int NB, int sp, int C, cudaStream_t st, bool pdl = false);
+int launch_attention(const float* qkv, __half* out, __half* out_lo, int lo_mode, int NB, int T, int C, cudaStream_t st,
+                     bool pdl = false);
+int launch_pack_predictions(const float* seg, const float* cont, float* out, int NB, long long V, int n_classes, cudaStream_t st,
+                            bool pdl = false);
+int launch_ncdhw_to_ndhwc_f16(const float* x, __half* y, int NB, int C, int Cpad, long long V, cudaStream_t st, bool pdl = false);
 
 }
```

New measurement: 16.32 million, median of 6. About the same (+1.0%).
